# FaspDevTeam/faspsolver

Measured on AMD Instinct MI355X. Metric: AMG-PCG solve DOF/s (3D 7-pt Poisson 256^3, classical AMG V(1,1) w-Jacobi + PCG, rtol 1e-8), higher is better.
Workload: dtype f64

## Files before the change

### faspsolver_amd/__init__.py

```python
import ctypes as C
import os
import subprocess

import numpy as np

from . import _types as T
from ._types import *

_HERE = os.path.dirname(os.path.abspath(__file__))
LIB_PATH = os.environ.get("FASP_HIP_LIB") or os.path.join(_HERE, "libfasp_hip.so")
_lib = None

EXPORTS = [
    "fasp_param_amg_init", "fasp_param_solver_init", "fasp_solver_dcsr_krylov_amg",
    "fasp_blas_dcsr_mxv", "fasp_blas_dcsr_aAxpy", "fasp_blas_darray_dotprod",
    "fasp_blas_darray_norm2", "fasp_blas_darray_norminf", "fasp_blas_darray_axpy",
    "fasp_blas_darray_axpby", "fasp_smoother_dcsr_jacobi",
    "fasp_blas_dbsr_mxv", "fasp_blas_dbsr_aAxpy", "fasp_dbsr_getdiaginv", "fasp_smoother_dbsr_jacobi1",
    "fasp_solver_dbsr_pcg", "fasp_solver_dbsr_pbcgs", "fasp_solver_dbsr_pgmres", "fasp_solver_dbsr_pvgmres",
    "fasp_solver_dbsr_pvfgmres", "fasp_hip_bsr_precond_setup", "fasp_hip_bsr_precond_fct", "fasp_hip_bsr_precond_free",
    "fasp_hip_param_input", "fasp_fwrapper_dcsr_krylov_amg_", "fasp_dcsrvec_read2", "fasp_dvec_read",
    "fasp_dbsr_read", "fasp_dcoo_read", "fasp_dcoo_read1", "fasp_dcoo_shift_read", "fasp_dmtx_read", "fasp_dmtxsym_read", "fasp_dvec_write", "fasp_dcsr_write_coo", "fasp_dcsrvec_write2", "fasp_fwrapper_dcsr_amg_", "fasp_fwrapper_dbsr_krylov_amg_", "fasp_hip_free_bsr", "fasp_hip_comm_selftest", "fasp_hip_amg_kernel_info", "fasp_hip_coarse_kernel_info", "fasp_hip_bsr_coarse_kernel_info", "fasp_hip_coding_selftest", "fasp_solver_amg", "fasp_solver_famg", "fasp_hip_amg_solve", "fasp_precond_diag", "fasp_precond_dbsr_diag", "fasp_solver_dcsr_itsolver", "fasp_solver_dcsr_krylov", "fasp_solver_dcsr_krylov_diag", "fasp_solver_dbsr_itsolver", "fasp_solver_dbsr_krylov", "fasp_solver_dbsr_krylov_diag", "fasp_hip_mxv_csr", "fasp_hip_mxv_bsr", "fasp_solver_matfree_init", "fasp_solver_pcg", "fasp_solver_pbcgs", "fasp_solver_pgcg", "fasp_solver_pminres", "fasp_solver_pgmres", "fasp_solver_pvgmres", "fasp_solver_pvfgmres", "fasp_solver_itsolver", "fasp_solver_krylov", "fasp_solver_dcsr_pcg", "fasp_solver_dcsr_pminres", "fasp_solver_dcsr_pgcg", "fasp_solver_dcsr_pgcr", "fasp_solver_dcsr_pbcgs", "fasp_solver_dcsr_pgmres", "fasp_solver_dcsr_pvgmres",
    "fasp_solver_dcsr_pvfgmres", "fasp_hip_precond_setup", "fasp_hip_precond_fct", "fasp_hip_precond_free",
    "fasp_hip_time_bsr_mxv", "fasp_solver_dbsr_krylov_amg", "fasp_hip_bsr_amg_create", "fasp_hip_bsr_amg_create_host",
    "fasp_hip_bsr_amg_destroy", "fasp_hip_bsr_amg_num_levels", "fasp_hip_bsr_amg_get_matrix",
    "fasp_hip_bsr_amg_get_diaginv", "fasp_hip_bsr_solve",
    "fasp_hip_set_device", "fasp_hip_device_count", "fasp_hip_device_identity", "fasp_hip_available",
    "fasp_hip_amg_create", "fasp_hip_amg_create_host", "fasp_hip_amg_upload",
    "fasp_hip_amg_destroy", "fasp_hip_amg_num_levels", "fasp_hip_amg_get_matrix",
    "fasp_hip_amg_get_cfmark", "fasp_hip_solve", "fasp_hip_set_rhs", "fasp_hip_set_guess",
    "fasp_hip_solve_resident", "fasp_hip_get_solution", "fasp_hip_device_synchronize",
    "fasp_hip_precond_amg",
    "fasp_hip_poisson7pt", "fasp_hip_aniso27pt", "fasp_hip_free_system", "fasp_hip_time_kernel", "fasp_hip_measure_ceilings", "fasp_hip_amg_publish", "fasp_hip_amg_attach", "fasp_hip_amg_unpublish",
    "fasp_precond_setup", "fasp_precond_amg", "fasp_precond_famg", "fasp_precond_amli", "fasp_precond_namli", "fasp_amg_data_create", "fasp_amg_data_free", "fasp_param_amg_to_prec", "fasp_param_prec_to_amg", "fasp_mem_free", "fasp_mem_calloc", "fasp_dvec_alloc", "fasp_dvec_set", "fasp_dvec_free", "fasp_dvec_create", "fasp_dcsr_create", "fasp_dcsr_free", "fasp_smoother_dcsr_gs", "fasp_smoother_dcsr_sor", "fasp_smoother_dcsr_L1diag",
    "fasp_hip_tune", "fasp_hip_comm_unique_id", "fasp_hip_comm_init", "fasp_hip_comm_finalize",
    "fasp_hip_comm_rank", "fasp_hip_comm_size", "fasp_hip_version", "fasp_hip_comm_init_shm",
    "fasp_hip_dist_plan", "fasp_hip_dist_level_info", "fasp_hip_dist_get_matrix",
    "fasp_hip_dist_get_list",
    "fasp_blas_dcsr_vmv", "fasp_blas_dcsr_mxv_agg", "fasp_blas_dcsr_aAxpy_agg", "fasp_blas_darray_ax",
    "fasp_blas_darray_axpyz", "fasp_blas_darray_norm1", "fasp_darray_cp", "fasp_darray_set", "fasp_dvec_isnan",
    "fasp_hip_time_matrix", "fasp_hip_bsr_dist_info", "fasp_hip_seq_schedule_selftest", "fasp_hip_seq_chain_selftest", "fasp_hip_cluster_order", "fasp_hip_permute_csr", "fasp_hip_comm_init_ipc", "fasp_hip_comm_stats", "fasp_hip_comm_timing", "fasp_hip_estream_selftest", "fasp_hip_sell_selftest", "fasp_hip_csr_plan", "fasp_hip_level_op", "fasp_hip_matrix_op", "fasp_hip_matrix_traits",
    "fasp_param_ilu_init", "fasp_ilu_data_create", "fasp_ilu_data_free", "fasp_mem_iludata_check", "fasp_ilu_dcsr_setup",
    "fasp_precond_ilu", "fasp_precond_ilu_forward", "fasp_precond_ilu_backward", "fasp_solver_dcsr_krylov_ilu",
    "fasp_solver_dcsr_krylov_ilu_M", "fasp_smoother_dcsr_ilu", "fasp_fwrapper_dcsr_krylov_ilu_",
    "fasp_hip_ilu_resident_count", "fasp_hip_ilu_time",
    "fasp_ilu_dbsr_setup", "fasp_precond_dbsr_ilu", "fasp_solver_dbsr_krylov_ilu", "fasp_smoother_dbsr_ilu",
    "fasp_fwrapper_dbsr_krylov_ilu_",
    "fasp_hip_bsr_amg_get_ilu", "fasp_hip_bsr_amg_ilu_info", "fasp_hip_bsr_amg_ilu_smooth_time",
    "fasp_hip_bsr_sweep", "fasp_hip_csr_sweep",
    "fasp_blas_dcsr_rap", "fasp_hip_dcsr_rap", "fasp_hip_rap_info", "fasp_hip_rap_device_count", "fasp_hip_rap_time",
    "fasp_dstr_create", "fasp_dstr_alloc", "fasp_dstr_free", "fasp_dstr_cp", "fasp_format_dstr_dcsr", "fasp_dstr_read",
    "fasp_blas_dstr_aAxpy", "fasp_blas_dstr_mxv", "fasp_precond_dstr_diag", "fasp_solver_dstr_pcg", "fasp_solver_dstr_pbcgs",
    "fasp_solver_dstr_pminres", "fasp_solver_dstr_pgmres", "fasp_solver_dstr_pvgmres", "fasp_solver_dstr_itsolver",
    "fasp_solver_dstr_krylov", "fasp_solver_dstr_krylov_diag", "fasp_hip_mxv_str", "fasp_hip_str_form", "fasp_hip_time_str_mxv",
    "fasp_ilu_dstr_setup0", "fasp_ilu_dstr_setup1", "fasp_precond_dstr_ilu0", "fasp_precond_dstr_ilu1", "fasp_solver_dstr_krylov_ilu",
    "fasp_hip_str_ilu_form", "fasp_hip_str_ilu_apply", "fasp_hip_time_str_ilu",
    "fasp_smoother_dstr_jacobi", "fasp_smoother_dstr_jacobi1", "fasp_smoother_dstr_gs", "fasp_smoother_dstr_gs1",
    "fasp_smoother_dstr_gs_ascend", "fasp_smoother_dstr_gs_descend", "fasp_smoother_dstr_gs_order", "fasp_smoother_dstr_gs_cf",
    "fasp_smoother_dstr_sor", "fasp_smoother_dstr_sor1", "fasp_smoother_dstr_sor_ascend", "fasp_smoother_dstr_sor_descend",
    "fasp_smoother_dstr_sor_order", "fasp_smoother_dstr_sor_cf",
    "fasp_hip_str_sweep", "fasp_hip_str_sweep_form", "fasp_hip_str_sweep_levels", "fasp_hip_time_str_sweep",
    "fasp_generate_diaginv_block", "fasp_smoother_dstr_swz", "fasp_precond_dstr_blockgs", "fasp_solver_dstr_krylov_blockgs",
    "fasp_hip_str_swz", "fasp_hip_str_swz_levels", "fasp_hip_time_str_swz",
    "fasp_param_swz_init", "fasp_dcsr_sympart", "fasp_dcsr_shift", "fasp_sparse_mis", "fasp_swz_dcsr_setup", "fasp_dcsr_swz_forward",
    "fasp_dcsr_swz_backward", "fasp_precond_swz", "fasp_swz_data_free", "fasp_solver_dcsr_krylov_swz",
    "fasp_hip_csr_swz_levels", "fasp_hip_csr_swz", "fasp_hip_csr_swz_resident_count", "fasp_hip_time_csr_swz",
    "fasp_hip_csr_swz_runs", "fasp_hip_amg_get_swz", "fasp_hip_amg_swz_info", "fasp_hip_amg_swz_sweep_time", "fasp_hip_amg_swz_levels",
]


def build(verbose=False):
    cmd = ["make", "-C", os.path.join(_HERE, "csrc")]
    if not verbose:
        cmd.insert(1, "-s")
    subprocess.run(cmd, check=True)


def lib():
    global _lib
    if _lib is not None:
        return _lib
    if not os.path.exists(LIB_PATH):
        build()
    L = C.CDLL(LIB_PATH)
    P = C.POINTER
    L.fasp_param_amg_init.argtypes = [P(T.AMG_param)]
    L.fasp_param_solver_init.argtypes = [P(T.ITS_param)]
    L.fasp_solver_dcsr_krylov_amg.argtypes = [P(T.dCSRmat), P(T.dvector), P(T.dvector),
                                              P(T.ITS_param), P(T.AMG_param)]
    L.fasp_blas_dcsr_mxv.argtypes = [P(T.dCSRmat), T.c_double_p, T.c_double_p]
    L.fasp_blas_dcsr_aAxpy.argtypes = [C.c_double, P(T.dCSRmat), T.c_double_p, T.c_double_p]
    for f in ("fasp_blas_darray_dotprod", "fasp_blas_darray_norm2", "fasp_blas_darray_norminf"):
        getattr(L, f).restype = C.c_double
    L.fasp_blas_darray_dotprod.argtypes = [C.c_int, T.c_double_p, T.c_double_p]
    L.fasp_blas_darray_norm2.argtypes = [C.c_int, T.c_double_p]
    L.fasp_blas_darray_norminf.argtypes = [C.c_int, T.c_double_p]
    L.fasp_blas_darray_axpy.argtypes = [C.c_int, C.c_double, T.c_double_p, T.c_double_p]
    L.fasp_blas_darray_axpby.argtypes = [C.c_int, C.c_double, T.c_double_p, C.c_double,
                                         T.c_double_p]
    L.fasp_blas_dcsr_vmv.restype = C.c_double
    L.fasp_blas_dcsr_vmv.argtypes = [P(T.dCSRmat), T.c_double_p, T.c_double_p]
    L.fasp_blas_dcsr_mxv_agg.argtypes = [P(T.dCSRmat), T.c_double_p, T.c_double_p]
    L.fasp_blas_dcsr_aAxpy_agg.argtypes = [C.c_double, P(T.dCSRmat), T.c_double_p, T.c_double_p]
    L.fasp_blas_darray_ax.argtypes = [C.c_int, C.c_double, T.c_double_p]
    L.fasp_blas_darray_axpyz.argtypes = [C.c_int, C.c_double, T.c_double_p, T.c_double_p, T.c_double_p]
    L.fasp_blas_darray_norm1.restype = C.c_double
    L.fasp_blas_darray_norm1.argtypes = [C.c_int, T.c_double_p]
    L.fasp_darray_cp.argtypes = [C.c_int, T.c_double_p, T.c_double_p]
    L.fasp_darray_set.argtypes = [C.c_int, T.c_double_p, C.c_double]
    L.fasp_hip_time_matrix.restype = C.c_double
    L.fasp_hip_time_matrix.argtypes = [P(T.dCSRmat), C.c_int, C.c_int, P(C.c_int)]
    L.fasp_dvec_isnan.restype = C.c_short
    L.fasp_dvec_isnan.argtypes = [P(T.dvector)]
    L.fasp_smoother_dcsr_jacobi.argtypes = [P(T.dvector), C.c_int, C.c_int, C.c_int,
                                            P(T.dCSRmat), P(T.dvector), C.c_int, C.c_double]
    L.fasp_blas_dbsr_mxv.argtypes = [P(T.dBSRmat), T.c_double_p, T.c_double_p]
    L.fasp_blas_dbsr_aAxpy.argtypes = [C.c_double, P(T.dBSRmat), T.c_double_p, T.c_double_p]
    L.fasp_dbsr_getdiaginv.argtypes = [P(T.dBSRmat)]
    L.fasp_dbsr_getdiaginv.restype = T.dvector
    L.fasp_smoother_dbsr_jacobi1.argtypes = [P(T.dBSRmat), P(T.dvector), P(T.dvector), T.c_double_p]
    L.fasp_hip_bsr_sweep.argtypes = [P(T.dBSRmat), T.c_double_p, T.c_double_p, T.c_double_p, C.c_int, C.c_int, C.c_double,
                                     P(C.c_int)]
    L.fasp_hip_csr_sweep.argtypes = [P(T.dCSRmat), P(C.c_int), C.c_int, C.c_int, C.c_double, C.c_int, T.c_double_p, T.c_double_p,
                                     P(C.c_int)]
    L.fasp_hip_time_bsr_mxv.argtypes = [P(T.dBSRmat), C.c_int]
    L.fasp_hip_time_bsr_mxv.restype = C.c_double
    L.fasp_solver_dcsr_pcg.argtypes = [P(T.dCSRmat), P(T.dvector), P(T.dvector), P(T.precond), C.c_double,
                                       C.c_double, C.c_int, C.c_short, C.c_short]
    L.fasp_solver_dcsr_pbcgs.argtypes = L.fasp_solver_dcsr_pcg.argtypes
    L.fasp_solver_dcsr_pminres.argtypes = L.fasp_solver_dcsr_pcg.argtypes
    L.fasp_solver_dcsr_pgcg.argtypes = L.fasp_solver_dcsr_pcg.argtypes
    L.fasp_solver_dcsr_pvgmres.argtypes = [P(T.dCSRmat), P(T.dvector), P(T.dvector), P(T.precond), C.c_double,
                                           C.c_double, C.c_int, C.c_short, C.c_short, C.c_short]
    L.fasp_solver_dcsr_pvfgmres.argtypes = L.fasp_solver_dcsr_pvgmres.argtypes
    L.fasp_solver_dcsr_pgmres.argtypes = L.fasp_solver_dcsr_pvgmres.argtypes
    L.fasp_solver_dcsr_pgcr.argtypes = L.fasp_solver_dcsr_pvgmres.argtypes
    L.fasp_hip_precond_setup.argtypes = [P(T.dCSRmat), P(T.AMG_param)]
    L.fasp_hip_precond_setup.restype = P(T.precond)
    L.fasp_hip_precond_free.argtypes = [P(T.precond)]
    L.fasp_hip_precond_free.restype = None
    L.fasp_hip_precond_fct.argtypes = [T.c_double_p, T.c_double_p, C.c_void_p]
    L.fasp_hip_precond_fct.restype = None
    L.fasp_solver_dbsr_pcg.argtypes = [P(T.dBSRmat), P(T.dvector), P(T.dvector), P(T.precond), C.c_double,
                                       C.c_double, C.c_int, C.c_short, C.c_short]
    L.fasp_solver_dbsr_pbcgs.argtypes = L.fasp_solver_dbsr_pcg.argtypes
    L.fasp_solver_dbsr_pvgmres.argtypes = [P(T.dBSRmat), P(T.dvector), P(T.dvector), P(T.precond), C.c_double,
                                           C.c_double, C.c_int, C.c_short, C.c_short, C.c_short]
    L.fasp_solver_dbsr_pgmres.argtypes = L.fasp_solver_dbsr_pvgmres.argtypes
    L.fasp_solver_dbsr_pvfgmres.argtypes = L.fasp_solver_dbsr_pvgmres.argtypes
    L.fasp_hip_bsr_precond_setup.argtypes = [P(T.dBSRmat), P(T.AMG_param)]
    L.fasp_hip_bsr_precond_setup.restype = P(T.precond)
    L.fasp_hip_bsr_precond_free.argtypes = [P(T.precond)]
    L.fasp_hip_bsr_precond_free.restype = None
    L.fasp_hip_bsr_precond_fct.argtypes = [T.c_double_p, T.c_double_p, C.c_void_p]
    L.fasp_hip_bsr_precond_fct.restype = None
    L.fasp_dcsrvec_read2.argtypes = [C.c_char_p, C.c_char_p, P(T.dCSRmat), P(T.dvector)]
    L.fasp_dvec_read.argtypes = [C.c_char_p, P(T.dvector)]
    L.fasp_dbsr_read.argtypes = [C.c_char_p, P(T.dBSRmat)]
    L.fasp_hip_free_bsr.argtypes = [P(T.dBSRmat)]
    L.fasp_hip_free_bsr.restype = None
    L.fasp_hip_param_input.argtypes = [C.c_char_p, P(T.ITS_param), P(T.AMG_param)]
    L.fasp_fwrapper_dcsr_krylov_amg_.argtypes = [P(C.c_int), P(C.c_int), T.c_int_p, T.c_int_p, T.c_double_p,
                                                 T.c_double_p, T.c_double_p, P(C.c_double), P(C.c_int), P(C.c_int)]
    L.fasp_fwrapper_dcsr_krylov_amg_.restype = None
    L.fasp_hip_coding_selftest.argtypes = [P(T.dCSRmat), P(C.c_int)]
    L.fasp_hip_amg_kernel_info.argtypes = [C.c_void_p, C.c_int, C.c_int, P(C.c_int), P(C.c_double)]
    L.fasp_hip_coarse_kernel_info.argtypes = [C.c_void_p, P(C.c_int)]
    L.fasp_hip_bsr_coarse_kernel_info.argtypes = [C.c_void_p, P(C.c_int)]
    L.fasp_solver_amg.argtypes = [P(T.dCSRmat), P(T.dvector), P(T.dvector), P(T.AMG_param)]
    L.fasp_hip_amg_solve.argtypes = [C.c_void_p, P(T.dvector), P(T.dvector), P(T.AMG_param), T.c_double_p,
                                     C.c_int, P(T.fasp_hip_stats)]
    L.fasp_solver_dbsr_krylov_amg.argtypes = [P(T.dBSRmat), P(T.dvector), P(T.dvector), P(T.ITS_param),
                                              P(T.AMG_param)]
    L.fasp_hip_bsr_amg_create.argtypes = [P(C.c_void_p), P(T.dBSRmat), P(T.AMG_param)]
    L.fasp_hip_bsr_amg_create_host.argtypes = [P(C.c_void_p), P(T.dBSRmat), P(T.AMG_param)]
    L.fasp_hip_bsr_amg_destroy.argtypes = [C.c_void_p]
    L.fasp_hip_bsr_amg_destroy.restype = None
    L.fasp_hip_bsr_amg_num_levels.argtypes = [C.c_void_p]
    L.fasp_hip_bsr_amg_get_matrix.argtypes = [C.c_void_p, C.c_int, C.c_int, P(T.dBSRmat)]
    L.fasp_hip_bsr_amg_get_diaginv.argtypes = [C.c_void_p, C.c_int]
    L.fasp_hip_bsr_amg_get_diaginv.restype = T.c_double_p
    L.fasp_hip_bsr_solve.argtypes = [C.c_void_p, P(T.dvector), P(T.dvector), P(T.ITS_param), T.c_double_p,
                                     C.c_int, P(T.fasp_hip_stats)]
    L.fasp_hip_amg_create.argtypes = [P(C.c_void_p), P(T.dCSRmat), P(T.AMG_param)]
    L.fasp_hip_amg_create_host.argtypes = L.fasp_hip_amg_create.argtypes
    L.fasp_hip_amg_upload.argtypes = [C.c_void_p]
    L.fasp_hip_amg_destroy.argtypes = [C.c_void_p]
    L.fasp_hip_amg_destroy.restype = None
    L.fasp_hip_amg_num_levels.argtypes = [C.c_void_p]
    L.fasp_hip_amg_get_matrix.argtypes = [C.c_void_p, C.c_int, C.c_int, P(T.dCSRmat)]
    L.fasp_hip_amg_get_cfmark.argtypes = [C.c_void_p, C.c_int, P(T.ivector)]
    L.fasp_hip_solve.argtypes = [C.c_void_p, P(T.dvector), P(T.dvector), P(T.ITS_param),
                                 T.c_double_p, C.c_int, P(T.fasp_hip_stats)]
    L.fasp_hip_set_rhs.argtypes = [C.c_void_p, P(T.dvector)]
    L.fasp_hip_set_guess.argtypes = [C.c_void_p, P(T.dvector)]
    L.fasp_hip_get_solution.argtypes = [C.c_void_p, P(T.dvector)]
    L.fasp_hip_solve_resident.argtypes = [C.c_void_p, P(T.ITS_param), T.c_double_p, C.c_int,
                                          P(T.fasp_hip_stats)]
    L.fasp_hip_precond_amg.argtypes = [C.c_void_p, T.c_double_p, T.c_double_p]
    L.fasp_hip_poisson7pt.argtypes = [C.c_int, C.c_int, C.c_int, P(T.dCSRmat), P(T.dvector),
                                      P(T.dvector)]
    L.fasp_hip_aniso27pt.argtypes = [C.c_int, C.c_double, C.c_double, C.c_double, P(T.dCSRmat), P(T.dvector)]
    L.fasp_hip_free_system.argtypes = [P(T.dCSRmat), P(T.dvector), P(T.dvector)]
    L.fasp_hip_free_system.restype = None
    L.fasp_hip_measure_ceilings.argtypes = [P(C.c_double), C.c_size_t, C.c_int]
    L.fasp_hip_amg_publish.argtypes = [C.c_void_p, C.c_char_p]
    L.fasp_hip_amg_attach.argtypes = [P(C.c_void_p), C.c_char_p]
    L.fasp_hip_amg_unpublish.argtypes = [C.c_char_p]
    L.fasp_hip_time_kernel.restype = C.c_double
    L.fasp_hip_time_kernel.argtypes = [C.c_void_p, C.c_int, C.c_int, C.c_int]
    L.fasp_hip_tune.argtypes = [C.c_char_p, C.c_int]
    L.fasp_hip_comm_unique_id.argtypes = [C.c_char_p]
    L.fasp_hip_comm_init.argtypes = [C.c_int, C.c_int, C.c_char_p]
    L.fasp_hip_version.restype = C.c_char_p
    L.fasp_hip_comm_init_shm.argtypes = [C.c_int, C.c_int, C.c_char_p]
    L.fasp_hip_dist_plan.argtypes = [C.c_void_p, C.c_int, C.c_int, C.c_int]
    L.fasp_hip_dist_level_info.argtypes = [C.c_void_p, C.c_int, T.c_int_p]
    L.fasp_hip_dist_get_matrix.argtypes = [C.c_void_p, C.c_int, C.c_int, P(T.dCSRmat)]
    L.fasp_hip_dist_get_list.argtypes = [C.c_void_p, C.c_int, C.c_int, P(T.ivector)]
    _lib = L
    L.fasp_param_ilu_init.argtypes = [P(T.ILU_param)]
    L.fasp_param_ilu_init.restype = None
    L.fasp_ilu_data_create.argtypes = [C.c_int, C.c_int, P(T.ILU_data)]
    L.fasp_ilu_data_create.restype = None
    L.fasp_ilu_data_free.argtypes = [P(T.ILU_data)]
    L.fasp_ilu_data_free.restype = None
    L.fasp_mem_iludata_check.argtypes = [P(T.ILU_data)]
    L.fasp_mem_iludata_check.restype = C.c_short
    L.fasp_ilu_dcsr_setup.argtypes = [P(T.dCSRmat), P(T.ILU_data), P(T.ILU_param)]
    L.fasp_ilu_dcsr_setup.restype = C.c_short
    for f in ("fasp_precond_ilu", "fasp_precond_ilu_forward", "fasp_precond_ilu_backward"):
        getattr(L, f).argtypes = [T.c_double_p, T.c_double_p, C.c_void_p]
        getattr(L, f).restype = None
    L.fasp_solver_dcsr_krylov_ilu.argtypes = [P(T.dCSRmat), P(T.dvector), P(T.dvector), P(T.ITS_param), P(T.ILU_param)]
    L.fasp_solver_dcsr_krylov_ilu_M.argtypes = [P(T.dCSRmat), P(T.dvector), P(T.dvector), P(T.ITS_param),
                                                P(T.ILU_param), P(T.dCSRmat)]
    L.fasp_smoother_dcsr_ilu.argtypes = [P(T.dCSRmat), P(T.dvector), P(T.dvector), C.c_void_p]
    L.fasp_smoother_dcsr_ilu.restype = None
    L.fasp_fwrapper_dcsr_krylov_ilu_.argtypes = [P(C.c_int), P(C.c_int), T.c_int_p, T.c_int_p, T.c_double_p,
                                                 T.c_double_p, T.c_double_p, P(C.c_double), P(C.c_int), P(C.c_int)]
    L.fasp_fwrapper_dcsr_krylov_ilu_.restype = None
    L.fasp_hip_ilu_time.argtypes = [P(T.ILU_data), C.c_int, C.c_int, T.c_double_p]
    L.fasp_hip_ilu_time.restype = C.c_double
    L.fasp_ilu_dbsr_setup.argtypes = [P(T.dBSRmat), P(T.ILU_data), P(T.ILU_param)]
    L.fasp_ilu_dbsr_setup.restype = C.c_short
    L.fasp_precond_dbsr_ilu.argtypes = [T.c_double_p, T.c_double_p, C.c_void_p]
    L.fasp_precond_dbsr_ilu.restype = None
    L.fasp_solver_dbsr_krylov_ilu.argtypes = [P(T.dBSRmat), P(T.dvector), P(T.dvector), P(T.ITS_param), P(T.ILU_param)]
    L.fasp_solver_dbsr_krylov_ilu.restype = C.c_int
# ... 264 lines not shown
    def publish(self, name):
        st = lib().fasp_hip_amg_publish(self.h, name.encode())
        if st < 0:
            raise RuntimeError(f"fasp_hip_amg_publish({name}) failed with status {st}")

    @staticmethod
    def unpublish(name):
        lib().fasp_hip_amg_unpublish(name.encode())

    @property
    def num_levels(self):
        return lib().fasp_hip_amg_num_levels(self.h)

    def upload(self):
        st = lib().fasp_hip_amg_upload(self.h)
        if st < 0:
            raise RuntimeError(f"fasp_hip_amg_upload failed with status {st}")

    def matrix(self, level, which):
        v = T.dCSRmat()
        st = lib().fasp_hip_amg_get_matrix(self.h, level, which, C.byref(v))
        if st < 0:
            raise IndexError((level, which))
        ia, ja, val = T.csr_arrays(v)
        return v.row, v.col, ia, ja, val

    def cfmark(self, level):
        v = T.ivector()
        if lib().fasp_hip_amg_get_cfmark(self.h, level, C.byref(v)) < 0:
            raise IndexError(level)
        return np.ctypeslib.as_array(v.val, (v.row,)).copy()

    def solve(self, b, itparam, x0=None, hist_cap=600):
        x = np.zeros(self.n) if x0 is None else np.ascontiguousarray(x0, dtype=np.float64).copy()
        bv, _b = T.as_vec(b)
        xv, x = T.as_vec(x)
        hist = np.zeros(hist_cap)
        stats = T.fasp_hip_stats()
        st = lib().fasp_hip_solve(self.h, C.byref(bv), C.byref(xv), C.byref(itparam),
                                  T.dp(hist), hist_cap, C.byref(stats))
        return st, x, hist[:max(stats.nhist, 0)].copy(), stats

    def amg_solve(self, b, amgparam=None, x0=None, hist_cap=600):
        x = np.zeros(self.n) if x0 is None else np.ascontiguousarray(x0, dtype=np.float64).copy()
        bv, _b = T.as_vec(b)
        xv, x = T.as_vec(x)
        hist = np.zeros(hist_cap)
        stats = T.fasp_hip_stats()
        st = lib().fasp_hip_amg_solve(self.h, C.byref(bv), C.byref(xv),
                                      C.byref(amgparam) if amgparam is not None else None,
                                      T.dp(hist), hist_cap, C.byref(stats))
        return st, x, hist[:max(min(stats.nhist, hist_cap), 0)].copy(), stats

    def set_rhs(self, b):
        bv, _b = T.as_vec(b)
        st = lib().fasp_hip_set_rhs(self.h, C.byref(bv))
        if st < 0:
            raise RuntimeError(f"fasp_hip_set_rhs failed: {st}")

    def solve_resident(self, itparam, hist_cap=600):
        st = lib().fasp_hip_set_guess(self.h, None)
        if st < 0:
            raise RuntimeError(f"fasp_hip_set_guess failed: {st}")
        hist = np.zeros(hist_cap)
        stats = T.fasp_hip_stats()
        st = lib().fasp_hip_solve_resident(self.h, C.byref(itparam), T.dp(hist), hist_cap,
                                           C.byref(stats))
        return st, hist[:max(stats.nhist, 0)].copy(), stats

    def get_solution(self):
        x = np.zeros(self.n)
        xv, x = T.as_vec(x)
        st = lib().fasp_hip_get_solution(self.h, C.byref(xv))
        if st < 0:
            raise RuntimeError(f"fasp_hip_get_solution failed: {st}")
        return x

    def kernel_info(self, level, which=0):
        k = C.c_int(0); b = C.c_double(0)
        if lib().fasp_hip_amg_kernel_info(self.h, level, which, C.byref(k), C.byref(b)) < 0:
            raise IndexError((level, which))
        return k.value, b.value

    def coarse_kernel_info(self):
        info = (C.c_int * 8)()
        if lib().fasp_hip_coarse_kernel_info(self.h, info) < 0:
            raise RuntimeError("fasp_hip_coarse_kernel_info failed")
        return tuple(info)

    def precond(self, r):
        r = np.ascontiguousarray(r, dtype=np.float64)
        z = np.zeros_like(r)
        st = lib().fasp_hip_precond_amg(self.h, T.dp(r), T.dp(z))
        if st < 0:
            raise RuntimeError(f"fasp_hip_precond_amg failed: {st}")
        return z

    def dist_plan(self, rank, nranks, min_rows):
        st = lib().fasp_hip_dist_plan(self.h, rank, nranks, min_rows)
        if st < 0:
            raise RuntimeError(f"fasp_hip_dist_plan failed: {st}")

    def dist_info(self, level):
        info = (C.c_int * 8)()
        if lib().fasp_hip_dist_level_info(self.h, level, info) < 0:
            raise IndexError(level)
        keys = ("replicated", "nglobal", "row0", "nloc", "nghost", "nsend", "first_replicated", "nranks")
        return dict(zip(keys, list(info)))

    def dist_matrix(self, level, which):
        v = T.dCSRmat()
        if lib().fasp_hip_dist_get_matrix(self.h, level, which, C.byref(v)) < 0:
            raise IndexError((level, which))
        ia, ja, val = T.csr_arrays(v)
        return v.row, v.col, ia, ja, val

    def dist_list(self, level, which):
        v = T.ivector()
        if lib().fasp_hip_dist_get_list(self.h, level, which, C.byref(v)) < 0:
            raise IndexError((level, which))
        if v.row == 0:
            return np.zeros(0, np.int32)
        return np.ctypeslib.as_array(v.val, (v.row,)).copy()

    def time_kernel(self, kind, level=0, reps=20):
        return lib().fasp_hip_time_kernel(self.h, kind, level, reps)

    def swz(self, level):
        d = T.SWZ_data()
        st = lib().fasp_hip_amg_get_swz(self.h, level, C.byref(d))
        if st < 0:
            raise IndexError(level)
        if st == 0:
            return None
        iblock = np.ctypeslib.as_array(d.iblock, (d.nblk + 1,)).copy()
        jblock = np.ctypeslib.as_array(d.jblock, (int(iblock[-1]),)).copy()
        n, nnz = d.A.row, d.A.nnz
        ia = np.ctypeslib.as_array(d.A.IA, (n + 1,)).copy()
        ja = np.ctypeslib.as_array(d.A.JA, (max(nnz, 1),))[:nnz].copy()
        val = np.ctypeslib.as_array(d.A.val, (max(nnz, 1),))[:nnz].copy()
        return dict(nblk=d.nblk, maxbs=d.maxbs, SWZ_type=d.SWZ_type, iblock=iblock, jblock=jblock, A=(ia, ja, val))

    def swz_levels(self, level):
        v = C.c_int(0)
        if lib().fasp_hip_amg_swz_levels(self.h, level, C.byref(v)) < 0:
            raise IndexError(level)
        return v.value

    def swz_info(self, level):
        info = (C.c_int * 8)()
        st = lib().fasp_hip_amg_swz_info(self.h, level, info)
        if st < 0:
            raise IndexError(level)
        if st == 0:
            return None
        keys = ("levels_fwd", "levels_bwd", "launches_fwd", "launches_bwd", "nblk", "maxbs", "nswap", "nfactor")
        return dict(zip(keys, list(info)))

    def swz_sweep_time(self, level, dir=0, reps=20):
        ms = lib().fasp_hip_amg_swz_sweep_time(self.h, level, dir, reps)
        if ms < 0:
            raise RuntimeError(f"fasp_hip_amg_swz_sweep_time failed: {int(ms)}")
        return ms

    def close(self):
        if self.h:
# ... 121 lines not shown
```

### faspsolver_amd/csrc/device_csr.hip.h

```cpp

struct DevCSR {
    int     row = 0, col = 0, nnz = 0;
    int*    ia  = nullptr;
    int*    ja  = nullptr;
    double* val = nullptr;
    int*    dpos = nullptr;
    bool    dup_diag = false;
    bool    sorted = false;
    int     lanes = 8;
    int     kind = 0;
    int     tile_rows = 256;
    int     wrows = 64, wcap = 512;
    unsigned char* code = nullptr;
    int*    rowbase = nullptr;
    int*    doff = nullptr;
    double* dval = nullptr;
    unsigned short* pat = nullptr;
    int*    pstart = nullptr;
    int*    plen = nullptr;
    int*    poff = nullptr;
    double* pval = nullptr;
    int     npat = 0, npent = 0;
    unsigned short* ja16 = nullptr;
    int*            jbase = nullptr;
    int     nxrows = -1;
    int     plane = 0;
    int     win_lo = 0, win_hi = -1;
    unsigned short* lja16 = nullptr;
    int*    tptr = nullptr;
    int*    tcols = nullptr;
    long long ntcols = 0;
    const int* bridge = nullptr;
    double*    bscratch = nullptr;
    int        bridge_dir = 0;
    int*       es_tab = nullptr;
    unsigned short* es_ja16 = nullptr;
    double*    es_part = nullptr;
    int        es_W = 0, es_nc = 0;
    unsigned*      sell_code = nullptr;
    int*           sell_meta = nullptr;
    unsigned char* sell_rlen = nullptr;
    double*        sell_tab = nullptr;
    int            sell_nv = 0, sell_obits = 0, sell_nslice = 0;
    long long      sell_slots = 0;
    void    release()
    {
        if (sell_code) (void)hipFree(sell_code);
        if (sell_meta) (void)hipFree(sell_meta);
        if (sell_rlen) (void)hipFree(sell_rlen);
        if (sell_tab) (void)hipFree(sell_tab);
        sell_code = nullptr; sell_meta = nullptr; sell_rlen = nullptr; sell_tab = nullptr; sell_nv = sell_obits = sell_nslice = 0; sell_slots = 0;
        if (es_tab) (void)hipFree(es_tab);
        if (es_part) (void)hipFree(es_part);
        if (es_ja16) (void)hipFree(es_ja16);
        es_tab = nullptr; es_part = nullptr; es_ja16 = nullptr; es_W = es_nc = 0;
        if (bscratch) (void)hipFree(bscratch);
        bscratch = nullptr; bridge = nullptr; bridge_dir = 0;
        if (lja16) (void)hipFree(lja16);
        if (tptr) (void)hipFree(tptr);
        if (tcols) (void)hipFree(tcols);
        lja16 = nullptr; tptr = nullptr; tcols = nullptr;
        nxrows = -1;
        if (ja16) (void)hipFree(ja16);
        ja16 = nullptr;
        if (jbase) (void)hipFree(jbase);
        jbase = nullptr;
        if (ia) (void)hipFree(ia);
        if (ja) (void)hipFree(ja);
        if (val) (void)hipFree(val);
        if (dpos) (void)hipFree(dpos);
        if (code) (void)hipFree(code);
        if (rowbase) (void)hipFree(rowbase);
        if (doff) (void)hipFree(doff);
        if (dval) (void)hipFree(dval);
        if (pat) (void)hipFree(pat);
        if (pstart) (void)hipFree(pstart);
        if (plen) (void)hipFree(plen);
        if (poff) (void)hipFree(poff);
        if (pval) (void)hipFree(pval);
        pat = nullptr; pstart = plen = poff = nullptr; pval = nullptr;
        ia = ja = dpos = rowbase = doff = nullptr; val = dval = nullptr; code = nullptr;
    }
};

static void pick_kernel(DevCSR& M)
{
    const double avg = M.row > 0 ? (double)M.nnz / M.row : 1.0;
    static const double stream_max = std::getenv("FASP_HIP_STREAM_MAX") ? std::atof(std::getenv("FASP_HIP_STREAM_MAX")) : 48.0;
    M.kind = avg <= stream_max ? 2 : 0;
    M.lanes = avg < 300.0 ? 16 : avg < 1000.0 ? 32 : 64;
    while (M.lanes < 64 && (double)M.row * M.lanes < 0.75 * MAXGRID * BLOCK) M.lanes *= 2;
    if (avg < 48.0) M.lanes = avg < 3.0 ? 2 : avg < 6.0 ? 4 : avg < 24.0 ? 8 : 16;
    static const int small_rows = std::getenv("FASP_HIP_SMALL_XFER_ROWS") ? std::atoi(std::getenv("FASP_HIP_SMALL_XFER_ROWS")) : 256 * 1024;
    if (M.kind == 2 && M.row != M.col && M.row < small_rows) M.kind = 0;
    int R = 256;
    while (R < STREAM_MAXR && R * 2 * avg <= 3072.0) R <<= 1;
    M.tile_rows = R;
    M.wrows = 64;
    M.wcap  = 512;
}

static bool g_oneshot_upload = false;
static bool compress_enabled()
{
    if (g_oneshot_upload) return false;
    static int en = -1;
    if (en < 0) { const char* e = std::getenv("FASP_HIP_COMPRESS"); en = (e && std::atoi(e) == 0) ? 0 : 1; }
    return en != 0;
}
struct PairKey { int off; unsigned long long bits; };
static inline unsigned pair_hash(int off, unsigned long long bits)
{
    unsigned long long h = bits * 0x9E3779B97F4A7C15ull + (unsigned long long)(unsigned)off * 0xC2B2AE3D27D4EB4Full;
    return (unsigned)(h >> 40);
}
static bool build_dict8(const HostCSR& M, std::vector<int>& doff, std::vector<double>& dval,
                        Buf<unsigned char>& code, Buf<int>& rowbase)
{
    const bool square = M.row == M.col;
    const int n = M.row;
    if (n <= 0 || M.nnz <= 0) return false;
    constexpr int SLOTS = 1024;
    struct Table {
        int      cnt = 0;
        int      slot_id[SLOTS];
        PairKey  keys[257];
        Table() { for (int& s : slot_id) s = -1; }
        int find_or_add(int off, unsigned long long bits, bool add)
        {
// ... 127 lines not shown
#pragma omp for schedule(static)
        for (int r = 0; r < n; ++r) {
            const unsigned long long h = row_hash(r);
            rh[r] = h;
            if (fail) continue;
            S->add(h, r);
            if (S->cnt > maxpat) fail = true;
        }
    }
    Set* Gs = nullptr;
    std::vector<std::pair<int, unsigned long long>> reps;
    if (!fail) {
        Gs = new Set(SLOTS);
        for (Set* S : local)
            if (S)
                for (int s = 0; s < SLOTS && !fail; ++s)
                    if (S->key[s]) { Gs->add(S->key[s], S->first[s]); if (Gs->cnt > maxpat) fail = true; }
    }
    for (Set* S : local) delete S;
    if (fail) { delete Gs; return false; }
    for (int s = 0; s < SLOTS; ++s)
        if (Gs->key[s]) reps.emplace_back(Gs->first[s], Gs->key[s]);
    std::sort(reps.begin(), reps.end());
    long long tot = 0;
    for (auto& q : reps) tot += (M.ia[q.first + 1] - M.ia[q.first] + 7) / 8 * 8;
    if (tot > MAXENT || (long long)reps.size() * 8 > n || tot * 4 > M.nnz) { delete Gs; return false; }
    pstart.assign(reps.size(), 0); plen.assign(reps.size(), 0);
    poff.clear(); pval.clear();
    for (size_t i = 0; i < reps.size(); ++i) {
        const int r = reps[i].first, base = base_of(r);
        pstart[i] = (int)poff.size();
        plen[i] = M.ia[r + 1] - M.ia[r];
        for (int k = M.ia[r]; k < M.ia[r + 1]; ++k) { poff.push_back(M.ja[k] - base); pval.push_back(M.val[k]); }
        while (poff.size() % 8) { poff.push_back(0); pval.push_back(0.0); }
    }
    for (int s = 0; s < SLOTS; ++s) Gs->first[s] = -1;
    {
        Set& S = *Gs;
        for (size_t i = 0; i < reps.size(); ++i) {
            unsigned s = (unsigned)(reps[i].second >> 20) & (SLOTS - 1);
            while (S.key[s] != reps[i].second) s = (s + 1) & (SLOTS - 1);
            S.first[s] = (int)i;
        }
    }
    pat.alloc((size_t)n);
    if (!square) rowbase.alloc((size_t)n);
    bool collision = false;
#pragma omp parallel for schedule(static) num_threads(nt)
    for (int r = 0; r < n; ++r) {
        const int id = Gs->find(rh[r]);
        if (id < 0 || !same_row(r, reps[(size_t)id].first)) { collision = true; continue; }
        pat[r] = (unsigned short)id;
        if (!square) rowbase[r] = base_of(r);
    }
    delete Gs;
    return !collision;
}

static int grid_plane_of(const std::vector<int>& poff, int nrow)
{
    constexpr int UNIT = 8 * 2 * BLOCK;
    std::vector<int> cand;
    for (int o : poff) {
        const long long m = std::llabs((long long)o);
        const long long c = (m + UNIT / 2) / UNIT * UNIT;
        if (c >= UNIT && c <= nrow / 4 && std::find(cand.begin(), cand.end(), (int)c) == cand.end() && cand.size() < 64) cand.push_back((int)c);
    }
    int best = 0;
    double best_cost = 0.2;
    for (int P : cand) {
        double cost = 0.0;
        for (int o : poff) {
            long long r = (long long)o % P;
            if (r > P / 2) r -= P;
            if (r < -P / 2) r += P;
            cost += (double)std::min<long long>(std::llabs(r), P / 8) / (P / 8);
        }
        cost /= std::max<size_t>(poff.size(), 1);
        if (cost < best_cost || (cost == best_cost && P > best)) { best_cost = cost; best = P; }
    }
    return best;
}

static bool rows_span_16bit(const int* ia, const int* ja, int row)
{
    int bad = 0;
#pragma omp parallel for schedule(static) reduction(+ : bad)
    for (int i = 0; i < row; ++i) {
        if (ia[i + 1] <= ia[i]) continue;
        int lo = ja[ia[i]], hi = lo;
        for (int k = ia[i] + 1; k < ia[i + 1]; ++k) { lo = std::min(lo, ja[k]); hi = std::max(hi, ja[k]); }
        if (hi - lo >= 65536) ++bad;
    }
    return bad == 0;
}
static int upload_ja16(DevCSR& D, const int* ia_host, const int* ja_dev_order)
{
    static const bool on = !(std::getenv("FASP_HIP_JA16") && std::atoi(std::getenv("FASP_HIP_JA16")) == 0);
    if (!on || D.kind != 0 || D.nnz < 4096) return FASP_SUCCESS;
    const bool relative = D.col > 65536;
    if (relative && !rows_span_16bit(ia_host, ja_dev_order, D.row)) return FASP_SUCCESS;
    Buf<unsigned short> j16((size_t)D.nnz);
    Buf<int> base(relative ? (size_t)D.row : 0);
#pragma omp parallel for schedule(static)
    for (int i = 0; i < D.row; ++i) {
        int lo = 0;
        if (relative) {
            lo = ia_host[i + 1] > ia_host[i] ? ja_dev_order[ia_host[i]] : 0;
            for (int k = ia_host[i]; k < ia_host[i + 1]; ++k) lo = std::min(lo, ja_dev_order[k]);
            base[(size_t)i] = lo;
        }
        for (int k = ia_host[i]; k < ia_host[i + 1]; ++k) j16[k] = (unsigned short)(ja_dev_order[k] - lo);
    }
    HIPCK(hipMalloc(&D.ja16, sizeof(unsigned short) * ((size_t)D.nnz + 8)));
    HIPCK(hipMemset(D.ja16 + D.nnz, 0, sizeof(unsigned short) * 8));
    HIPCK(hipMemcpy(D.ja16, j16.data(), sizeof(unsigned short) * (size_t)D.nnz, hipMemcpyHostToDevice));
    if (relative) {
        HIPCK(hipMalloc(&D.jbase, sizeof(int) * (size_t)D.row));
        HIPCK(hipMemcpy(D.jbase, base.data(), sizeof(int) * (size_t)D.row, hipMemcpyHostToDevice));
    }
    return FASP_SUCCESS;
}

static int g_device_sort = 1;
constexpr int SORT_BLK = 256, SORT_MAXLEN = 16384;
__global__ __launch_bounds__(SORT_BLK) void k_sort_rows(int nrow, const int* __restrict__ ia, const int* __restrict__ ja_in,
                                                        const double* __restrict__ val_in, int* __restrict__ ja_out,
                                                        double* __restrict__ val_out, unsigned short* __restrict__ ja16, int* __restrict__ jbase)
{
    extern __shared__ unsigned long long sort_keys[];
    const int tid = threadIdx.x;
    for (int r = blockIdx.x; r < nrow; r += gridDim.x) {
        const int kb = ia[r], len = ia[r + 1] - kb;
        int P = 1;
        while (P < len) P <<= 1;
        for (int i = tid; i < P; i += SORT_BLK)
            sort_keys[i] = i < len ? ((unsigned long long)(unsigned)ja_in[kb + i] << 32) | (unsigned)i : ~0ull;
        __syncthreads();
        for (int k = 2; k <= P; k <<= 1)
            for (int j = k >> 1; j > 0; j >>= 1) {
                for (int t = tid; t < P / 2; t += SORT_BLK) {
                    const int i = ((t & ~(j - 1)) << 1) | (t & (j - 1)), l = i | j;
                    const unsigned long long a = sort_keys[i], b = sort_keys[l];
                    if ((a > b) == ((i & k) == 0)) { sort_keys[i] = b; sort_keys[l] = a; }
                }
                __syncthreads();
            }
        const int base = (jbase && len > 0) ? (int)(sort_keys[0] >> 32) : 0;
        if (jbase && tid == 0) jbase[r] = base;
        for (int i = tid; i < len; i += SORT_BLK) {
            const unsigned long long key = sort_keys[i];
            const int col = (int)(key >> 32);
            ja_out[kb + i] = col;
            val_out[kb + i] = val_in[kb + (int)(unsigned)key];
            if (ja16) ja16[kb + i] = (unsigned short)(col - base);
        }
        __syncthreads();
    }
}

static int upload_sorted_on_device(const HostCSR& H, DevCSR& D, int maxlen)
{
    static const bool ja16_on = !(std::getenv("FASP_HIP_JA16") && std::atoi(std::getenv("FASP_HIP_JA16")) == 0);
    int* tj = nullptr; double* tv = nullptr;
    HIPCK(hipMalloc(&tj, sizeof(int) * (size_t)H.nnz));
    if (hipMalloc(&tv, sizeof(double) * (size_t)H.nnz) != hipSuccess) { (void)hipFree(tj); return ERROR_ALLOC_MEM; }
// ... 357 lines not shown
#pragma omp parallel for schedule(static)
    for (int s = 0; s < ns; ++s) {
        const int W = S.sptr[(size_t)s + 1] - S.sptr[(size_t)s], base = S.sbase[(size_t)s];
        unsigned* cs = S.code.data() + (size_t)S.sptr[(size_t)s] * 64;
        for (int l = 0; l < 64; ++l) {
            const int r = s * 64 + l;
            const int kb = r < n ? M.ia[r] : 0, len = r < n ? M.ia[r + 1] - kb : 0;
            for (int k = 0; k < len; ++k) {
                const int sl = Gs.slot(bits_of(M.val[kb + k]));
                if (sl < 0) { lost = true; continue; }
                const int id = Gs.id[(size_t)sl];
                cs[(size_t)k * 64 + l] = ((unsigned)id << S.obits) | (unsigned)(M.ja[kb + k] - base);
            }
            for (int k = len; k < W; ++k) cs[(size_t)k * 64 + l] = 0u;
        }
    }
    if (lost) { why = 4; return false; }
    why = 0;
    return true;
}

static void sell_mxv_host(const SellHost& S, int nrow, const double* x, double* y)
{
    const unsigned omask = (1u << S.obits) - 1u;
    for (int s = 0; s < S.nslice; ++s) {
        const int W = S.sptr[(size_t)s + 1] - S.sptr[(size_t)s], base = S.sbase[(size_t)s];
        const unsigned* cs = S.code.data() + (size_t)S.sptr[(size_t)s] * 64;
        double acc[64];
        for (int l = 0; l < 64; ++l) acc[l] = 0.0;
        for (int k = 0; k < W; ++k)
            for (int l = 0; l < 64; ++l) {
                const int r = s * 64 + l;
                if (r >= nrow || k >= (int)S.rlen[(size_t)r]) continue;
                const unsigned c = cs[(size_t)k * 64 + l];
                acc[l] = acc[l] + S.tab[c >> S.obits] * x[base + (int)(c & omask)];
            }
        for (int l = 0; l < 64 && s * 64 + l < nrow; ++l) y[s * 64 + l] = acc[l];
    }
}
static void sell_decode_host(const SellHost& S, int nrow, int* ia, int* ja, double* val)
{
    const unsigned omask = (1u << S.obits) - 1u;
    ia[0] = 0;
    for (int r = 0; r < nrow; ++r) ia[r + 1] = ia[r] + (int)S.rlen[(size_t)r];
    for (int r = 0; r < nrow; ++r) {
        const int s = r >> 6, l = r & 63, base = S.sbase[(size_t)s];
        const unsigned* cs = S.code.data() + (size_t)S.sptr[(size_t)s] * 64;
        for (int k = 0; k < (int)S.rlen[(size_t)r]; ++k) {
            const unsigned c = cs[(size_t)k * 64 + l];
            ja[ia[r] + k] = base + (int)(c & omask);
            val[ia[r] + k] = S.tab[c >> S.obits];
        }
    }
}

static int upload_sell(const HostCSR& H, DevCSR& D)
{
    static const bool on = !(std::getenv("FASP_HIP_SELL") && std::atoi(std::getenv("FASP_HIP_SELL")) == 0);
    if (!on) return FASP_SUCCESS;
    static const bool timing = std::getenv("FASP_HIP_SETUP_TIMING") != nullptr;
    const double t0 = wall_seconds();
    SellHost S;
    int why = 0;
    const bool ok = build_sell(H, S, SELL_CAP_PERCENT, &why);
    if (timing) std::printf("        [sell %d x %d, %d nnz] %s (%d) %d values, %d + %d bits, %.3f slots per entry, %.3f s\n", H.row, H.col, H.nnz,
                            ok ? "coded" : "not coded", why, S.nv, S.vbits, S.obits, (double)S.slots / std::max(H.nnz, 1), wall_seconds() - t0);
    if (!ok) return FASP_SUCCESS;
    const size_t ns = (size_t)S.nslice;
    std::vector<int> meta(2 * ns + 1);
    std::copy(S.sptr.begin(), S.sptr.end(), meta.begin());
    std::copy(S.sbase.begin(), S.sbase.end(), meta.begin() + (long)ns + 1);
    HIPCK(hipMalloc(&D.sell_code, sizeof(unsigned) * (size_t)std::max<long long>(S.slots, 1)));
    HIPCK(hipMalloc(&D.sell_meta, sizeof(int) * meta.size()));
    HIPCK(hipMalloc(&D.sell_rlen, (size_t)H.row));
    HIPCK(hipMalloc(&D.sell_tab, sizeof(double) * (size_t)S.nv));
    HIPCK(hipMemcpy(D.sell_code, S.code.data(), sizeof(unsigned) * (size_t)S.slots, hipMemcpyHostToDevice));
    HIPCK(hipMemcpy(D.sell_meta, meta.data(), sizeof(int) * meta.size(), hipMemcpyHostToDevice));
    HIPCK(hipMemcpy(D.sell_rlen, S.rlen.data(), (size_t)H.row, hipMemcpyHostToDevice));
    HIPCK(hipMemcpy(D.sell_tab, S.tab.data(), sizeof(double) * (size_t)S.nv, hipMemcpyHostToDevice));
    D.sell_nv = S.nv; D.sell_obits = S.obits; D.sell_nslice = S.nslice; D.sell_slots = S.slots;
    return FASP_SUCCESS;
}

static int upload_csr(const HostCSR& H, DevCSR& D)
{
    D.row = H.row; D.col = H.col; D.nnz = H.nnz;
    HIPCK(hipMalloc(&D.ia, sizeof(int) * ((size_t)H.row + 1)));
    HIPCK(hipMalloc(&D.ja, sizeof(int) * std::max<size_t>(H.nnz, 1)));
    HIPCK(hipMalloc(&D.val, sizeof(double) * (std::max<size_t>(H.nnz, 1) + 2)));
    HIPCK(hipMemsetAsync(D.val + std::max<size_t>(H.nnz, 1), 0, sizeof(double) * 2, g_ctx.stream));
    HIPCK(hipMemcpyAsync(D.ia, H.ia.data(), sizeof(int) * ((size_t)H.row + 1), hipMemcpyHostToDevice, g_ctx.stream));
    pick_kernel(D);
    auto upload_plain = [&]() -> int {
        HIPCK(hipMemcpyAsync(D.ja, H.ja.data(), sizeof(int) * (size_t)H.nnz, hipMemcpyHostToDevice, g_ctx.stream));
        HIPCK(hipMemcpyAsync(D.val, H.val.data(), sizeof(double) * (size_t)H.nnz, hipMemcpyHostToDevice, g_ctx.stream));
        return 0;
    };
    if (compress_enabled() && H.nnz >= 4096 && (double)H.nnz <= 48.0 * H.row) {
        Buf<unsigned short> pat; Buf<int> prb;
        std::vector<int> pstart, plen, poff; std::vector<double> pval;
        static const bool rowpat_on = !(std::getenv("FASP_HIP_ROWPAT") && std::atoi(std::getenv("FASP_HIP_ROWPAT")) == 0);
        if (rowpat_on && build_rowpat(H, pat, pstart, plen, poff, pval, prb)) {
            D.npat = (int)pstart.size(); D.npent = (int)poff.size();
            HIPCK(hipMalloc(&D.pat, sizeof(unsigned short) * ((size_t)H.row + 2)));
            HIPCK(hipMalloc(&D.pstart, sizeof(int) * pstart.size()));
            HIPCK(hipMalloc(&D.plen, sizeof(int) * plen.size()));
            HIPCK(hipMemcpy(D.plen, plen.data(), sizeof(int) * plen.size(), hipMemcpyHostToDevice));
            HIPCK(hipMalloc(&D.poff, sizeof(int) * std::max<size_t>(poff.size(), 1)));
            HIPCK(hipMalloc(&D.pval, sizeof(double) * std::max<size_t>(pval.size(), 1)));
            HIPCK(hipMemset(D.pat + H.row, 0xff, sizeof(unsigned short) * 2));
            HIPCK(hipMemcpy(D.pat, pat.data(), sizeof(unsigned short) * (size_t)H.row, hipMemcpyHostToDevice));
            HIPCK(hipMemcpy(D.pstart, pstart.data(), sizeof(int) * pstart.size(), hipMemcpyHostToDevice));
            HIPCK(hipMemcpy(D.poff, poff.data(), sizeof(int) * poff.size(), hipMemcpyHostToDevice));
            HIPCK(hipMemcpy(D.pval, pval.data(), sizeof(double) * pval.size(), hipMemcpyHostToDevice));
            if (prb.n) {
                HIPCK(hipMalloc(&D.rowbase, sizeof(int) * ((size_t)H.row + 2)));
                HIPCK(hipMemcpy(D.rowbase, prb.data(), sizeof(int) * (size_t)H.row, hipMemcpyHostToDevice));
                const int nr = H.row, npair = (nr + 1) / 2;
                long long nx = 0;
#pragma omp parallel for schedule(static) reduction(+ : nx)
                for (int w0 = 0; w0 < nr; w0 += 128) {
                    const int    pm = std::min((w0 + 64) / 2, npair - 1);
                    const unsigned domA = pat[(size_t)2 * pm], domB = (2 * pm + 1 < nr) ? pat[(size_t)2 * pm + 1] : 0xffffu;
                    for (int r = w0; r < std::min(w0 + 128, nr); r += 2) {
                        const bool vb = r + 1 < nr;
                        if (!(vb && pat[r] == domA && pat[r + 1] == domB)) nx += vb ? 2 : 1;
                    }
                }
                if (nx * 4 <= nr) D.nxrows = (int)nx;
            } else {
                D.plane = grid_plane_of(poff, H.row);
                if (std::getenv("FASP_HIP_SETUP_TIMING")) std::printf("        [upload_csr %d x %d, %d nnz] %d row patterns; grid plane for the XCD strips: %d rows\n", H.row, H.col, H.nnz, (int)pstart.size(), D.plane);
                const int nr = H.row, npair = (nr + 1) / 2;
                long long nx = 0;
#pragma omp parallel for schedule(static) reduction(+ : nx)
                for (int w0 = 0; w0 < nr; w0 += 128) {
                    const unsigned dom = pat[(size_t)2 * std::min((w0 + 64) / 2, npair - 1)];
                    for (int r = w0; r < std::min(w0 + 128, nr); r += 2) {
                        const bool vb = r + 1 < nr;
                        if (!(vb && pat[r] == dom && pat[r + 1] == dom)) nx += vb ? 2 : 1;
                    }
                }
                if (nx * 4 <= nr) D.nxrows = (int)nx;
            }
            D.kind = 2;
            return upload_plain() < 0 ? ERROR_ALLOC_MEM : FASP_SUCCESS;
        }
        std::vector<int> doff; std::vector<double> dval;
        Buf<unsigned char> code; Buf<int> rowbase;
        if (build_dict8(H, doff, dval, code, rowbase)) {
            HIPCK(hipMalloc(&D.code, (size_t)H.nnz + 256));
            HIPCK(hipMalloc(&D.doff, sizeof(int) * 256));
            HIPCK(hipMalloc(&D.dval, sizeof(double) * 256));
            HIPCK(hipMemcpy(D.code, code.data(), (size_t)H.nnz, hipMemcpyHostToDevice));
            HIPCK(hipMemcpy(D.doff, doff.data(), sizeof(int) * 256, hipMemcpyHostToDevice));
            HIPCK(hipMemcpy(D.dval, dval.data(), sizeof(double) * 256, hipMemcpyHostToDevice));
            if (rowbase.n) {
                HIPCK(hipMalloc(&D.rowbase, sizeof(int) * (size_t)H.row));
                HIPCK(hipMemcpy(D.rowbase, rowbase.data(), sizeof(int) * (size_t)H.row, hipMemcpyHostToDevice));
            }
            D.kind = 2;
            return upload_plain() < 0 ? ERROR_ALLOC_MEM : FASP_SUCCESS;
        }
    }
    static const bool sort_long = !(std::getenv("FASP_HIP_SORT_LONG_ROWS") && std::atoi(std::getenv("FASP_HIP_SORT_LONG_ROWS")) == 0);
    static const int  sort_stream = std::getenv("FASP_HIP_SORT_STREAM") ? std::atoi(std::getenv("FASP_HIP_SORT_STREAM")) : 0;
    const double avg_len = H.row > 0 ? (double)H.nnz / H.row : 0.0;
    const bool do_sort = sort_long && !g_oneshot_upload && H.nnz > 0 && (D.kind == 0 || (D.kind == 2 && sort_stream > 0 && avg_len >= sort_stream));
    static const bool timing = std::getenv("FASP_HIP_SETUP_TIMING") != nullptr;
    double tp = wall_seconds();
    auto lap = [&](const char* what) {
        if (!timing) return;
        const double now = wall_seconds();
        std::printf("        [upload_csr %d x %d, %d nnz] %-10s %8.3f s\n", H.row, H.col, H.nnz, what, now - tp);
        tp = now;
    };
    if (do_sort && D.kind == 0) {
        int maxlen = 0;
#pragma omp parallel for schedule(static) reduction(max : maxlen)
        for (int i = 0; i < H.row; ++i) maxlen = std::max(maxlen, H.ia[i + 1] - H.ia[i]);
        if (g_device_sort && maxlen <= SORT_MAXLEN) {
            const int st = upload_sorted_on_device(H, D, maxlen);
            lap("device sort");
            return st < 0 ? st : build_estream(H.ia.data(), H.row, H.nnz, D);
        }
    }
    if (do_sort) {
        Buf<int> sj((size_t)H.nnz);
        Buf<double> sv((size_t)H.nnz);
        std::vector<int> dp;
        const bool square = H.row == H.col;
        if (square) dp.assign((size_t)H.row, -1);
#pragma omp parallel
        {
            std::vector<std::pair<int, double>> tmp;
#pragma omp for schedule(dynamic, 64)
            for (int i = 0; i < H.row; ++i) {
                const int kb = H.ia[i], ke = H.ia[i + 1];
                tmp.resize((size_t)(ke - kb));
                for (int k = kb; k < ke; ++k) tmp[(size_t)(k - kb)] = {H.ja[k], H.val[k]};
                std::stable_sort(tmp.begin(), tmp.end(),
                                 [](const std::pair<int, double>& x, const std::pair<int, double>& y) { return x.first < y.first; });
                for (int k = kb; k < ke; ++k) {
                    sj[k] = tmp[(size_t)(k - kb)].first; sv[k] = tmp[(size_t)(k - kb)].second;
                    if (square && sj[k] == i) dp[(size_t)i] = k;
                }
            }
        }
        lap("row sort");
        HIPCK(hipMemcpy(D.ja, sj.data(), sizeof(int) * (size_t)H.nnz, hipMemcpyHostToDevice));
        HIPCK(hipMemcpy(D.val, sv.data(), sizeof(double) * (size_t)H.nnz, hipMemcpyHostToDevice));
        lap("memcpy");
        if (square && D.kind == 2) {
            HIPCK(hipMalloc(&D.dpos, sizeof(int) * (size_t)std::max(H.row, 1)));
            HIPCK(hipMemcpy(D.dpos, dp.data(), sizeof(int) * (size_t)H.row, hipMemcpyHostToDevice));
        }
        D.sorted = true;
        if (upload_ja16(D, H.ia.data(), sj.data()) < 0) return ERROR_ALLOC_MEM;
        return build_estream(H.ia.data(), H.row, H.nnz, D);
    }
    if (upload_plain() < 0) return ERROR_ALLOC_MEM;
    if (D.kind == 2 && !g_oneshot_upload && build_xtile(H, D) < 0) return ERROR_ALLOC_MEM;
    if (D.kind == 2 && compress_enabled() && upload_sell(H, D) < 0) return ERROR_ALLOC_MEM;
    if (upload_ja16(D, H.ia.data(), H.ja.data()) < 0) return ERROR_ALLOC_MEM;
    return build_estream(H.ia.data(), H.row, H.nnz, D);
}

struct Tuning { int swz_run = -1, swz_run_width = 16, ilu_smooth_fused = 1, gen2 = 2, ws2_bpc = 3, maxgrid = -1, xcd = 16, nt = 1, kind = -1, lanes = -1, wrows = -1, wcap = -1, compress = 1, rpl = -1, lds_tab = 1, xcd_pat = 64, spcg_batch = 16, small_lds = 1, ja16 = 1, spcg_fused = 1, spcg_grid = 0, spcg_persist = 1, split_rows = 0, gs_multicolor = 0, seq_flow = 1, seq_strip_kb = 0, seq_jobs = 1, seq_spine = 1, seq_grid = 0, seq_chain = 1, seq_chain_n1 = 0, seq_chain_grid = 0, seq_chain_ref = 0, seq_test_hang = 0, seq_rest_lanes = 0, local_square = 1, fuse_zr = 1, fuse_presmooth = 1, seq_lanes = 0, xtile = 1, rp5_max = 45, rp_bpc = 5, rp_xcd = -1, rp_strip = 2, spcg_test_hang = 0, small_onewave = 4, lazy_coarse = 1, rp_stream = -1, renumber = 1, renumber_chunk = 262144, pcg_dev_beta = 1, spcg_spec = 1, ev_every = 4, pcg_fold = 1, seq_chain_touch = 8, seq_chain_touch_t1 = 1, seq_zero_skip = 1, estream = 1, es_dbg = 0, ilu_form = -1, str_ilu_form = -1, str_ilu_wgs = 0, str_sweep_form = -1, str_sweep_wgs = 0, sell = 1; };
static Tuning g_tune;

template <class K>
static int resident_blocks_per_cu(K kernel)
{
    static std::vector<std::pair<const void*, int>> cache;
    const void* key = reinterpret_cast<const void*>(kernel);
    for (const auto& e : cache)
        if (e.first == key) return e.second;
    int nb = 0;
    if (hipOccupancyMaxActiveBlocksPerMultiprocessor(&nb, kernel, BLOCK, 0) != hipSuccess || nb < 1) nb = 4;
    nb = std::min(nb, 8);
    cache.emplace_back(key, nb);
    return nb;
}

template <class K>
static int launch_persistent(K kernel, int ntiles, CsrArgs& a, int blocks_per_cu = 0)
{
    int cap = (blocks_per_cu > 0 ? std::min(blocks_per_cu, resident_blocks_per_cu(kernel)) : resident_blocks_per_cu(kernel)) * g_ctx.num_cu;
    if (g_tune.maxgrid > 0) cap = g_tune.maxgrid;
    cap = std::min(cap, MAXGRID);
    int grid = std::min(cap, ntiles);
    grid = std::max(8, (grid + 7) / 8 * 8);
    hipLaunchKernelGGL(kernel, dim3(grid), dim3(BLOCK), 0, g_ctx.stream, a);
    return grid;
}

enum CsrKernel : int {
    CK_ROWS_2 = 0, CK_ROWS_4, CK_ROWS_8, CK_ROWS_16, CK_ROWS_32, CK_ROWS_64,
    CK_WSTREAM_64_512, CK_WSTREAM_64_1024, CK_WSTREAM_32_512, CK_WSTREAM_32_1024,
    CK_ROWPAT_0_1, CK_ROWPAT_0_2, CK_ROWPAT_1_1, CK_ROWPAT_1_2, CK_ROWPAT_2_1, CK_ROWPAT_2_2,
    CK_DICT8_8, CK_DICT8_16, CK_DICT8_24,
    CK_ESTREAM_4, CK_ESTREAM_8, CK_ESTREAM_16, CK_ESTREAM_32,
    CK_ROWPAT4, CK_ROWPAT5, CK_LSTREAM, CK_XTILE, CK_SELL, CK_WSTREAM2
};
struct CsrPlan {
    CsrKernel kernel;
    int    family;
    int    tile_rows;
    int    bpc;
    int    xcd_map;
    int    tpp;
    int    nt;
    bool   ja16, jbase;
    bool   fused_zr;
    double bytes;
};
static CsrPlan plan_csr(const DevCSR& M, int op, bool windowed, bool want_partials, int rows = -1)
{
    CsrPlan p{};
    int kind = M.kind;
    if (rows < 0) rows = M.row;
    if (M.code && g_tune.compress) kind = 4;
    if (M.pat && g_tune.compress) kind = 5;
    if (g_tune.kind >= 0 && !(g_tune.kind == 4 && !M.code) && !(g_tune.kind == 5 && !M.pat)) kind = g_tune.kind;
    const int lanes = g_tune.lanes > 0 ? g_tune.lanes : M.lanes, wrows = g_tune.wrows > 0 ? g_tune.wrows : M.wrows, wcap = g_tune.wcap > 0 ? g_tune.wcap : M.wcap;
    const bool jac = op == OP_JACOBI, w64 = wrows == 64 && wcap == 512;
    const bool lstream_ok = g_tune.gen2 && kind == 2 && w64 && (double)M.nnz <= 7.6 * M.row;
    if (jac && kind != 0 && kind < 4 && (M.dup_diag || !M.dpos) && !lstream_ok) kind = 0;
    p.xcd_map = g_tune.xcd;
    p.nt = g_tune.nt | ((g_tune.rp_stream > 0 || (g_tune.rp_stream < 0 && (size_t)M.row * 8 > (size_t)96 << 20)) ? 4 : 0);
    p.ja16 = g_tune.ja16 && M.ja16; p.jbase = g_tune.ja16 && M.jbase;
    if (M.jbase && kind != 0) p.ja16 = p.jbase = false;
    if (kind == 1 || kind == 3) kind = 0;
    p.tile_rows = kind >= 4 ? BLOCK : kind == 2 ? 4 * wrows : BLOCK / lanes;
    auto ntiles = [&] { return (rows + p.tile_rows - 1) / p.tile_rows; };
    auto strips = [&] {
        const int rpb = p.tile_rows;
        if (!g_tune.rp_strip || M.plane < 8 * rpb || M.plane % (8 * rpb) != 0 || ntiles() < 4 * (M.plane / rpb)) return;
        p.xcd_map = -2; p.tpp = M.plane / rpb;
    };
    const double avg = M.row > 0 ? (double)M.nnz / M.row : 1.0, ptr_bytes = 4.0 * (M.row + 1.0), base_bytes = M.rowbase ? 4.0 * M.row : 0.0;
    const bool pair = kind == 5 && M.nxrows >= 0 && g_tune.rpl <= 0;
    p.bytes = kind == 5 ? 2.0 * M.row + base_bytes + 12.0 * M.npent : kind == 4 ? 1.0 * M.nnz + ptr_bytes + base_bytes : 12.0 * M.nnz + ptr_bytes;
    if (pair && g_tune.gen2 && !M.rowbase) {
        p.kernel = CK_ROWPAT4; p.family = 6; p.tile_rows = 2 * BLOCK;
        p.xcd_map = ntiles() >= 8 * 64 ? g_tune.rp_xcd : 16;
        if (p.xcd_map == -1) strips();
        p.bpc = p.xcd_map == -2 && g_tune.rp_bpc == 5 ? 3 : g_tune.rp_bpc;
        p.fused_zr = jac && want_partials;
    }
    else if (pair && g_tune.gen2 >= 2 && M.rowbase && !jac && op != OP_L1DIAG && (double)M.nnz <= 0.1 * g_tune.rp5_max * M.row) {
        p.kernel = CK_ROWPAT5; p.family = 9; p.tile_rows = 2 * BLOCK; p.bpc = 5;
        p.xcd_map = ntiles() >= 8 * 64 ? -1 : 16;
        if (g_tune.rp_strip >= 2) strips();
    }
    else if (kind == 5) {
        const int rpl = g_tune.rpl > 0 ? g_tune.rpl : 1;
        const bool lds = M.npat <= 512 && M.npent <= 2048 && g_tune.lds_tab != 0;
        const int T = !lds ? 0 : M.npat <= 64 && M.npent <= 512 && g_tune.lds_tab != 3 ? 2 : 1;
        p.kernel = CsrKernel(CK_ROWPAT_0_1 + 2 * T + (rpl != 1)); p.family = 5; p.tile_rows = BLOCK * rpl;
        if (g_tune.xcd_pat != 0) p.xcd_map = g_tune.xcd_pat;
        if (g_tune.xcd_pat == 64 && g_tune.rp_strip >= 2) strips();
    }
    else if (kind == 4) { p.kernel = avg <= 8.5 ? CK_DICT8_8 : avg <= 20.0 ? CK_DICT8_16 : CK_DICT8_24; p.family = 4; }
    else if (lstream_ok) { p.kernel = CK_LSTREAM; p.family = 7; p.bpc = 4; p.fused_zr = jac && want_partials; }
    else if (kind == 2 && g_tune.gen2 >= 2 && w64) {
        if (g_tune.xtile && M.lja16) {
            p.kernel = CK_XTILE; p.family = 10; p.bpc = 3;
            p.bytes = 10.0 * M.nnz + ptr_bytes + 4.0 * M.ntcols + 4.0 * ((M.row + 63) / 64 + 1.0);
        }
        else if (M.sell_code && g_tune.compress && g_tune.sell) {
            p.kernel = CK_SELL; p.family = 11; p.tile_rows = SELL_BLOCK;
            p.bytes = 4.0 * (double)M.sell_slots + 1.0 * M.row + 4.0 * (2.0 * M.sell_nslice + 1.0) + 8.0 * M.sell_nv;
        }
        else { p.kernel = CK_WSTREAM2; p.family = 8; p.bpc = g_tune.ws2_bpc; }
        p.fused_zr = jac && want_partials;
    }
    else if (kind == 2) {
        p.kernel = w64 ? CK_WSTREAM_64_512 : wrows == 64 ? CK_WSTREAM_64_1024 : wrows == 32 && wcap == 512 ? CK_WSTREAM_32_512 : CK_WSTREAM_32_1024; p.family = 2;
    }
    else {
        if (p.ja16) p.bytes = 10.0 * M.nnz + ptr_bytes + (p.jbase ? 4.0 * M.row : 0.0);
        const bool es_rule = g_tune.estream >= 2 || (g_tune.estream == 1 && (double)M.nnz < 256.0 * M.row);
        if (M.es_tab && es_rule && p.ja16 && !windowed && op != OP_MXV_DOT && !(jac && (want_partials || M.dup_diag)))
            p.kernel = avg >= 512.0 ? CK_ESTREAM_32 : avg >= 256.0 ? CK_ESTREAM_16 : avg >= 128.0 ? CK_ESTREAM_8 : CK_ESTREAM_4;
        else
            p.kernel = lanes == 2 ? CK_ROWS_2 : lanes == 4 ? CK_ROWS_4 : lanes == 8 ? CK_ROWS_8 : lanes == 16 ? CK_ROWS_16 : lanes == 32 ? CK_ROWS_32 : CK_ROWS_64;
    }
    return p;
}
static int kernel_family(const DevCSR& M, double* matrix_bytes)
{
    const CsrPlan p = plan_csr(M, OP_MXV, false, false);
    if (matrix_bytes) *matrix_bytes = p.bytes;
    return p.family;
}

template <int OP>
static int launch_sell(const DevCSR& M, CsrArgs& a)
{
    a.sell_code = M.sell_code; a.sell_sptr = M.sell_meta; a.sell_sbase = M.sell_meta + M.sell_nslice + 1; a.sell_rlen = M.sell_rlen;
    a.sell_tab = M.sell_tab; a.sell_nv = M.sell_nv; a.sell_obits = M.sell_obits;
    const size_t lds = sizeof(double) * ((size_t)M.sell_nv + SELL_NW);
    static bool attr_set = false;
    if (!attr_set) {
        (void)hipFuncSetAttribute(reinterpret_cast<const void*>(k_csr_sell<OP>), hipFuncAttributeMaxDynamicSharedMemorySize, (int)(sizeof(double) * (SELL_MAXV + SELL_NW)));
        attr_set = true;
    }
    static std::vector<std::pair<size_t, int>> cache;
    int nb = 0;
    for (const auto& e : cache)
        if (e.first == lds) nb = e.second;
    if (nb == 0) {
        if (hipOccupancyMaxActiveBlocksPerMultiprocessor(&nb, k_csr_sell<OP>, SELL_BLOCK, lds) != hipSuccess || nb < 1) nb = 1;
        nb = std::min(nb, 2);
        cache.emplace_back(lds, nb);
    }
    int cap = nb * g_ctx.num_cu;
    if (g_tune.maxgrid > 0) cap = g_tune.maxgrid;
    cap = std::min(cap, MAXGRID);
    int grid = std::min(cap, a.ntiles);
    grid = std::max(8, (grid + 7) / 8 * 8);
    hipLaunchKernelGGL(k_csr_sell<OP>, dim3(grid), dim3(SELL_BLOCK), lds, g_ctx.stream, a);
    return grid;
}

template <int OP>
static int launch_rowpat5(CsrArgs& a)
{
    if constexpr (OP == OP_JACOBI || OP == OP_L1DIAG) { (void)a; return 0; }
    else return launch_persistent(k_csr_rowpat5<OP>, a.ntiles, a, 5);
}

constexpr int WIN_ALIGN = DIST_WIN_ALIGN;
struct RowWin { int lo = 0, hi = -1, goff = 0; };

__global__ __launch_bounds__(BLOCK) void k_bridge_gather(int n, const int* __restrict__ perm, const double* __restrict__ s, double* __restrict__ y,
                                                         double* __restrict__ zx, const double* __restrict__ zdiag, double zomega)
{
    for (int k = blockIdx.x * BLOCK + threadIdx.x; k < n; k += gridDim.x * BLOCK) {
        const double v = s[perm[k]];
        y[k] = v;
        if (zx) { const double di = zdiag[k]; zx[k] = (fabs(di) > 1e-20) ? (1 - zomega) * 0.0 + zomega * v / di : 0.0; }
    }
}
__global__ __launch_bounds__(BLOCK) void k_bridge_scatter(int n, const int* __restrict__ perm, const double* __restrict__ x, double* __restrict__ s)
{
    for (int k = blockIdx.x * BLOCK + threadIdx.x; k < n; k += gridDim.x * BLOCK) s[perm[k]] = x[k];
}

template <int OP>
static int launch_csr(const DevCSR& M0, CsrArgs a, RowWin win = RowWin())
{
    if (M0.bridge && win.hi < 0) {
        DevCSR Mn = M0;
        Mn.bridge = nullptr; Mn.bscratch = nullptr; Mn.bridge_dir = 0;
        if (M0.bridge_dir == 1 && OP == OP_MXV) {
            CsrArgs b = a;
            b.y = M0.bscratch; b.zx = nullptr; b.zdiag = nullptr;
            const int G = launch_csr<OP>(Mn, b);
            const int grid = std::max(1, std::min(MAXGRID, (M0.row + BLOCK - 1) / BLOCK));
            hipLaunchKernelGGL(k_bridge_gather, dim3(grid), dim3(BLOCK), 0, g_ctx.stream, M0.row, M0.bridge, (const double*)M0.bscratch, a.y, a.zx, a.zdiag, a.zomega);
            return G;
        }
        if (M0.bridge_dir == 2 && (OP == OP_ADD || OP == OP_SUB || OP == OP_AXPY || OP == OP_MXV)) {
            const int grid = std::max(1, std::min(MAXGRID, (M0.col + BLOCK - 1) / BLOCK));
            hipLaunchKernelGGL(k_bridge_scatter, dim3(grid), dim3(BLOCK), 0, g_ctx.stream, M0.col, M0.bridge, a.x, M0.bscratch);
            CsrArgs b = a;
            b.x = M0.bscratch;
            return launch_csr<OP>(Mn, b);
        }
        std::fprintf(stderr, "### ERROR: fasp_hip: operation %d on a transfer operator with a numbering bridge (direction %d)\n", (int)OP, M0.bridge_dir);
        std::abort();
    }
    if (win.hi < 0 && g_tune.split_rows > 0 && M0.row >= 4 * WIN_ALIGN) {
        const int lo = std::min(g_tune.split_rows, M0.row / 4) / WIN_ALIGN * WIN_ALIGN, hi = (M0.row - lo) / WIN_ALIGN * WIN_ALIGN;
        RowWin w; w.lo = lo; w.hi = hi; w.goff = 0;
        int G = launch_csr<OP>(M0, a, w);
        w.lo = 0; w.hi = lo; w.goff = G;
        G += launch_csr<OP>(M0, a, w);
        w.lo = hi; w.hi = M0.row; w.goff = G;
        return G + launch_csr<OP>(M0, a, w);
    }
    const DevCSR& M = M0;
    const int w_lo = win.hi >= 0 ? win.lo : 0, w_hi = win.hi >= 0 ? std::min(win.hi, M0.row) : M0.row;
    if (w_hi <= w_lo && win.hi >= 0) return 0;
    if (a.partials) a.partials += win.goff;
    const CsrPlan p = plan_csr(M, OP, win.hi >= 0 || g_tune.split_rows > 0, a.partials != nullptr, w_hi - w_lo);
    const int rpb = p.tile_rows;
    if (win.hi >= 0 && rpb > 0 && (w_lo % rpb) != 0) {
        std::fprintf(stderr, "### ERROR: fasp_hip: row window at %d with a kernel tile of %d rows (a tuning knob broke the window alignment)\n", w_lo, rpb);
        std::abort();
    }
    a.nrow = w_hi; a.row_lo = w_lo; a.tile0 = w_lo / rpb;
    a.ntiles = (w_hi - w_lo + rpb - 1) / rpb; a.tiles_per_xcd = (a.ntiles + 7) / 8;
    a.xcd_map = p.xcd_map; a.nt = p.nt;
    if (p.tpp) { a.tpp = p.tpp; a.tiles_per_xcd = p.tpp / 8; }
    a.ia = M.ia; a.ja = M.ja; a.val = M.val; a.dpos = M.dpos;
    a.ja16 = p.ja16 ? M.ja16 : nullptr; a.jbase = p.jbase ? M.jbase : nullptr;
    if (p.family == 5 || p.family == 6 || p.family == 9) {
        a.pat = M.pat; a.pstart = M.pstart; a.plen = M.plen; a.poff = M.poff; a.pval = M.pval; a.rowbase = M.rowbase;
        a.npat = M.npat; a.npent = M.npent; a.ncol = M.col;
    }
    if (p.family == 4) { a.code = M.code; a.rowbase = M.rowbase; a.doff = M.doff; a.dval = M.dval; }
    if (p.kernel == CK_XTILE) { a.lja16 = M.lja16; a.tptr = M.tptr; a.tcols = M.tcols; }
#define PERSIST(...) return launch_persistent(__VA_ARGS__, a.ntiles, a, p.bpc)
    switch (p.kernel) {
        case CK_ROWS_2:  PERSIST(k_csr_rows<2, OP>);
        case CK_ROWS_4:  PERSIST(k_csr_rows<4, OP>);
        case CK_ROWS_8:  PERSIST(k_csr_rows<8, OP>);
        case CK_ROWS_16: PERSIST(k_csr_rows<16, OP>);
        case CK_ROWS_32: PERSIST(k_csr_rows<32, OP>);
        case CK_ROWS_64: PERSIST(k_csr_rows<64, OP>);
        case CK_WSTREAM_64_512:  PERSIST(k_csr_wstream<OP, 64, 512>);
        case CK_WSTREAM_64_1024: PERSIST(k_csr_wstream<OP, 64, 1024>);
        case CK_WSTREAM_32_512:  PERSIST(k_csr_wstream<OP, 32, 512>);
        case CK_WSTREAM_32_1024: PERSIST(k_csr_wstream<OP, 32, 1024>);
        case CK_ROWPAT_0_1: PERSIST(k_csr_rowpat<OP, 0, 1>);
        case CK_ROWPAT_0_2: PERSIST(k_csr_rowpat<OP, 0, 2>);
        case CK_ROWPAT_1_1: PERSIST(k_csr_rowpat<OP, 1, 1>);
        case CK_ROWPAT_1_2: PERSIST(k_csr_rowpat<OP, 1, 2>);
        case CK_ROWPAT_2_1: PERSIST(k_csr_rowpat<OP, 2, 1>);
        case CK_ROWPAT_2_2: PERSIST(k_csr_rowpat<OP, 2, 2>);
        case CK_DICT8_8:  PERSIST(k_csr_dict8<OP, 8>);
        case CK_DICT8_16: PERSIST(k_csr_dict8<OP, 16>);
        case CK_DICT8_24: PERSIST(k_csr_dict8<OP, 24>);
        case CK_ROWPAT4:  PERSIST(k_csr_rowpat4<OP>);
        case CK_ROWPAT5:  return launch_rowpat5<OP>(a);
        case CK_LSTREAM:  PERSIST(k_csr_lstream<OP, 512>);
        case CK_XTILE:    PERSIST(k_csr_xtile<OP>);
        case CK_SELL:     return launch_sell<OP>(M, a);
        case CK_WSTREAM2: PERSIST(k_csr_wstream2<OP>);
        default: break;
    }
#undef PERSIST
    const int W = M.es_W, nc = M.es_nc, lanes = 4 << (p.kernel - CK_ESTREAM_4);
    a.es_wc = M.es_tab; a.es_centry = a.es_wc + W + 1; a.es_crow = a.es_centry + nc + 1; a.es_hw0 = a.es_crow + nc + 1; a.es_np = a.es_hw0 + W;
    a.es_part = M.es_part; a.es_cnt = reinterpret_cast<unsigned*>(M.es_part + 2 * (size_t)W);
    a.es_cbase = M.es_ja16 ? a.es_np + W : nullptr; a.es_ja16 = M.es_ja16;
    static bool attr_set = false;
#define ES_ATTR(LL) (void)hipFuncSetAttribute(reinterpret_cast<const void*>(k_csr_estream<LL, OP>), hipFuncAttributeMaxDynamicSharedMemorySize, ES_LDS_BYTES)
    if (!attr_set) { ES_ATTR(32); ES_ATTR(16); ES_ATTR(8); ES_ATTR(4); attr_set = true; }
#undef ES_ATTR
#define ES_LAUNCH(LL) hipLaunchKernelGGL((k_csr_estream<LL, OP>), dim3(W / 4), dim3(BLOCK), ES_LDS_BYTES, g_ctx.stream, a)
#ifdef FASP_LAB_DEBUG
    if (OP == OP_MXV && g_tune.es_dbg) {
#define ES_DBG(LL, DD) do { (void)hipFuncSetAttribute(reinterpret_cast<const void*>(k_csr_estream<LL, OP_MXV, DD>), hipFuncAttributeMaxDynamicSharedMemorySize, ES_LDS_BYTES); hipLaunchKernelGGL((k_csr_estream<LL, OP_MXV, DD>), dim3(W / 4), dim3(BLOCK), ES_LDS_BYTES, g_ctx.stream, a); } while (0)
        const int dd = g_tune.es_dbg;
        if (lanes == 32) { if (dd == 1) ES_DBG(32, 1); else if (dd == 2) ES_DBG(32, 2); else if (dd == 3) ES_DBG(32, 3); else if (dd == 4) ES_DBG(32, 4); else ES_DBG(32, 7); }
        else if (lanes == 16) { if (dd == 1) ES_DBG(16, 1); else if (dd == 2) ES_DBG(16, 2); else if (dd == 3) ES_DBG(16, 3); else if (dd == 4) ES_DBG(16, 4); else ES_DBG(16, 7); }
        else if (lanes == 8) { if (dd == 1) ES_DBG(8, 1); else if (dd == 2) ES_DBG(8, 2); else if (dd == 3) ES_DBG(8, 3); else if (dd == 4) ES_DBG(8, 4); else ES_DBG(8, 7); }
        else { if (dd == 1) ES_DBG(4, 1); else if (dd == 2) ES_DBG(4, 2); else if (dd == 3) ES_DBG(4, 3); else if (dd == 4) ES_DBG(4, 4); else ES_DBG(4, 7); }
#undef ES_DBG
        return W / 4;
    }
#endif
    static const bool es_log = std::getenv("FASP_HIP_ES_LOG") != nullptr;
    if (es_log) { std::fprintf(stderr, "[es rank %d] op %d rows %d cols %d nnz %d W %d chunks %d lanes %d rel %d x %p y %p b %p\n", comm_rank(), (int)OP, M.row, M.col, M.nnz, W, nc, lanes, M.es_ja16 != nullptr, (const void*)a.x, (void*)a.y, (const void*)a.b); std::fflush(stderr); }
    if (lanes == 32) ES_LAUNCH(32); else if (lanes == 16) ES_LAUNCH(16); else if (lanes == 8) ES_LAUNCH(8); else ES_LAUNCH(4);
#undef ES_LAUNCH
    if (es_log) { const hipError_t e = hipStreamSynchronize(g_ctx.stream); std::fprintf(stderr, "[es rank %d] done: %s\n", comm_rank(), hipGetErrorString(e)); std::fflush(stderr); }
    return W / 4;
}

static void d_mxv(const DevCSR& A, const double* x, double* y)
{
    CsrArgs a{}; a.x = x; a.y = y;
    launch_csr<OP_MXV>(A, a);
}
static void d_resid(const DevCSR& A, const double* x, const double* b, double* y)
{
    CsrArgs a{}; a.x = x; a.y = y; a.b = b;
    launch_csr<OP_RESID>(A, a);
}
static void d_aAxpy(double alpha, const DevCSR& A, const double* x, double* y)
{
    CsrArgs a{}; a.x = x; a.y = y; a.alpha = alpha;
    if (alpha == 1.0) launch_csr<OP_ADD>(A, a);
    else if (alpha == -1.0) launch_csr<OP_SUB>(A, a);
    else launch_csr<OP_AXPY>(A, a);
}

static void d_finalize_to(int G, int nq, unsigned maxmask, double* out, bool dist)
{
    hipLaunchKernelGGL(k_finalize, dim3(1), dim3(BLOCK), 0, g_ctx.stream, g_ctx.d_partials, G, nq,
// ... 50 lines not shown
```

### faspsolver_amd/csrc/hierarchy.hip.h

```cpp

struct DevLevel {
    DevCSR  A, P, R;
    double* diag = nullptr;
    double* l1   = nullptr;
    double *b = nullptr, *xa = nullptr, *xb = nullptr, *w = nullptr;
    double* x  = nullptr;
    double* xo = nullptr;
    bool    x_zero = true;
    bool    presmoothed = false;
    double* halo_pending = nullptr;
    bool    owns_b = true;
    bool    replicated = true;
    int     nloc = 0;
    int     nvec = 0;
    int     row0 = 0;
    int     nglobal = 0;
    std::vector<int> send_off, recv_off;
    int*    d_send_idx = nullptr;
    double* d_sendbuf  = nullptr;
    bool    has_halo() const { return !replicated && nvec > nloc; }
    struct Sched {
        bool built = false, multicolor = false; int* d_order = nullptr; int* d_ptr = nullptr; std::vector<int> ptr;
        int ns = 0, L = 1, LR = 1, pfmax = 1, kt = 0, par = 1, nstrips = 0, nchunk = 0, maxent = 0; bool nolower = false, flow_ok = false, rowlevels = false, independent = false; int nrows = 0, nvirt = 0, nclasses = 0; long long nghost = 0, slot_bytes = 0;
        std::vector<int> cptr;
// ... 213 lines not shown
        (void)launch_csr<OP>(M, a);
        return -1;
    }
    RowWin w;
    w.lo = M.win_lo; w.hi = M.win_hi; w.goff = 0;
    int G = launch_csr<OP>(M, a, w);
    const int hst = halo_exchange(V, v, g_ctx.comm_stream);
    if (hipEventRecord(g_ctx.ev_halo, g_ctx.comm_stream) != hipSuccess ||
        hipStreamWaitEvent(g_ctx.stream, g_ctx.ev_halo, 0) != hipSuccess) {
        comm_mark_failed();
        (void)hipStreamSynchronize(g_ctx.comm_stream);
        local_ok = false;
    }
    w.lo = 0; w.hi = M.win_lo; w.goff = G;
    G += launch_csr<OP>(M, a, w);
    w.lo = M.win_hi; w.hi = M.row; w.goff = G;
    G += launch_csr<OP>(M, a, w);
    return (hst < 0 || !local_ok) ? -1 : G;
}

static bool renumber_param_ok(const AMG_param& p)
{
    return (p.smoother == SMOOTHER_JACOBI || p.smoother == SMOOTHER_L1DIAG) &&
           (p.cycle_type == V_CYCLE || p.cycle_type == W_CYCLE || p.cycle_type == VW_CYCLE || p.cycle_type == WV_CYCLE) &&
           p.coarse_scaling != 1 && p.AMG_type == CLASSIC_AMG;
}
static bool renumber_allowed(const fasp_hip_amg* h)
{
    if (g_oneshot_upload) return false;
    return g_tune.renumber != 0 && comm_size() == 1 && renumber_param_ok(h->param);
}
static int renumber_conflict(const fasp_hip_amg* h, const AMG_param& p)
{
    bool any = false;
    for (const auto& pm : h->perm) any = any || !pm.empty();
    if (!any || renumber_param_ok(p)) return FASP_SUCCESS;
    std::printf("### ERROR: fasp_hip: this hierarchy was uploaded for an order-independent smoother (its mid levels are renumbered); "
                "smoother %d / cycle %d / coarse_scaling %d need the natural order -- set them before the setup, or "
                "fasp_hip_tune(\"renumber\", 0)\n", (int)p.smoother, (int)p.cycle_type, (int)p.coarse_scaling);
    return ERROR_INPUT_PAR;
}
static bool dev_coded(const DevCSR& M) { return M.pat != nullptr || M.code != nullptr; }

static int upload_transfer(fasp_hip_amg* h, int l, const DistLevel* DLp)
{
    const HostLevel& HL = h->H.L[l];
    DevLevel& D = h->L[l];
    const bool rep = !DLp || DLp->replicated;
    const std::vector<int>* pf = (size_t)l < h->perm.size() && !h->perm[(size_t)l].empty() ? &h->perm[(size_t)l] : nullptr;
    const std::vector<int>* pc = (size_t)l + 1 < h->perm.size() && !h->perm[(size_t)l + 1].empty() ? &h->perm[(size_t)l + 1] : nullptr;
    const bool bridged = pc && !pf && dev_coded(D.A);
    if (bridged) {
        if (upload_csr(HL.P, D.P) < 0) return ERROR_ALLOC_MEM;
        if (upload_csr(HL.R, D.R) < 0) return ERROR_ALLOC_MEM;
        DevLevel& C = h->L[(size_t)l + 1];
        if (!C.d_perm) {
            HIPCK(hipMalloc(&C.d_perm, sizeof(int) * pc->size()));
            HIPCK(hipMemcpy(C.d_perm, pc->data(), sizeof(int) * pc->size(), hipMemcpyHostToDevice));
        }
        HIPCK(hipMalloc(&D.R.bscratch, sizeof(double) * pc->size()));
        HIPCK(hipMalloc(&D.P.bscratch, sizeof(double) * pc->size()));
        D.R.bridge = C.d_perm; D.R.bridge_dir = 1;
        D.P.bridge = C.d_perm; D.P.bridge_dir = 2;
    } else if (pf || pc) {
        std::vector<int> invf, invc;
        if (pf) { invf.resize(pf->size()); for (size_t k = 0; k < pf->size(); ++k) invf[(size_t)(*pf)[k]] = (int)k; }
        if (pc) { invc.resize(pc->size()); for (size_t k = 0; k < pc->size(); ++k) invc[(size_t)(*pc)[k]] = (int)k; }
        HostCSR T;
        permute_csr(HL.P, pf ? pf->data() : nullptr, pc ? invc.data() : nullptr, T);
        if (upload_csr(T, D.P) < 0) return ERROR_ALLOC_MEM;
        HIPCK(hipStreamSynchronize(g_ctx.stream));
        permute_csr(HL.R, pc ? pc->data() : nullptr, pf ? invf.data() : nullptr, T);
        if (upload_csr(T, D.R) < 0) return ERROR_ALLOC_MEM;
        HIPCK(hipStreamSynchronize(g_ctx.stream));
    } else {
        if (upload_csr(rep ? HL.P : DLp->P, D.P) < 0) return ERROR_ALLOC_MEM;
        if (upload_csr(rep ? HL.R : DLp->R, D.R) < 0) return ERROR_ALLOC_MEM;
    }
    if (D.A.plane > 0 && D.R.row > 0 && D.R.col > 0) {
        D.P.plane = D.A.plane;
        const long long pr = (long long)D.A.plane * D.R.row;
        if (pr % D.R.col == 0) D.R.plane = (int)(pr / D.R.col);
    }
    if (!rep) {
        D.R.win_lo = DLp->winR[0]; D.R.win_hi = DLp->winR[1];
        D.P.win_lo = DLp->winP[0]; D.P.win_hi = DLp->winP[1];
    }
    return FASP_SUCCESS;
}

static int upload_level(fasp_hip_amg* h, int l, const DistLevel* DLp)
{
    const HostLevel& HL = h->H.L[l];
    DevLevel& D = h->L[l];
    const bool rep = !DLp || DLp->replicated;
    D.replicated = rep;
    D.nloc = rep ? HL.A.row : DLp->nloc; D.row0 = rep ? 0 : DLp->row0; D.nglobal = HL.A.row;
    D.nvec = rep ? HL.A.row : DLp->nloc + (int)DLp->ghosts.size();
    const HostCSR& A = rep ? HL.A : DLp->A;
    static const bool timing = std::getenv("FASP_HIP_SETUP_TIMING") != nullptr;
    double tp = wall_seconds();
    auto lap = [&](const char* what) {
        if (!timing) return;
        const double now = wall_seconds();
        std::printf("    [upload level %d] %-10s %8.3f s\n", l, what, now - tp);
        tp = now;
    };
    const bool renum = renumber_allowed(h);
    if (h->perm.size() < h->L.size()) h->perm.resize(h->L.size());
    HostCSR Aperm;
    const HostCSR* Adev = &A;
    if (!rep && g_tune.local_square) {
        HostCSR view;
        view.row = A.row; view.col = A.col; view.nnz = A.nnz; view.row_aligned = true;
        view.ia.view(const_cast<int*>(A.ia.data()), A.ia.n); view.ja.view(const_cast<int*>(A.ja.data()), A.ja.n); view.val.view(const_cast<double*>(A.val.data()), A.val.n);
        if (upload_csr(view, D.A) < 0) return ERROR_ALLOC_MEM;
    } else {
        bool want = renum && rep && l > 0 && HL.has_coarse && !HL.SWZ && A.row >= 4096 && A.row <= 2000000 && (g_tune.renumber >= 2 || !dev_coded(h->L[(size_t)l - 1].A));
        bool uploaded = false;
        if (want && compress_enabled() && (double)A.nnz <= 48.0 * A.row) {
            if (upload_csr(A, D.A) < 0) return ERROR_ALLOC_MEM;
            if (dev_coded(D.A)) { want = false; uploaded = true; }
            else { HIPCK(hipStreamSynchronize(g_ctx.stream)); D.A.release(); D.A = DevCSR(); }
        }
        if (want) {
            std::vector<int>& pm = h->perm[(size_t)l];
            cluster_order(A, std::max(4096, g_tune.renumber_chunk), pm);
            std::vector<int> inv(pm.size());
            for (size_t k = 0; k < pm.size(); ++k) inv[(size_t)pm[k]] = (int)k;
            permute_csr(A, pm.data(), inv.data(), Aperm);
            Adev = &Aperm;
            lap("renumber");
        }
        if (!uploaded && upload_csr(*Adev, D.A) < 0) return ERROR_ALLOC_MEM;
    }
    lap("A");
    if (renum) {
        if (l > 0 && h->H.L[(size_t)l - 1].has_coarse && !h->L[(size_t)l - 1].P.ia) {
            const int st = upload_transfer(h, l - 1, nullptr);
            if (st < 0) return st;
            lap("P, R of the level above");
        }
    } else if (HL.has_coarse) {
        const int st = upload_transfer(h, l, DLp);
        if (st < 0) return st;
        lap("P, R");
    }
    if (!rep) { D.A.win_lo = DLp->winA[0]; D.A.win_hi = DLp->winA[1]; }
    HIPCK(hipStreamSynchronize(g_ctx.stream));
    lap("sync");
    if (upload_diag(*Adev, D) < 0) return ERROR_ALLOC_MEM;
    lap("diag");
    { const int st = swz_level_upload(h, l); if (st < 0) return st; }
    lap("Schwarz");
    const size_t n = D.nvec;
    if (l > 0) { if (alloc_vec(&D.b, n) < 0) return ERROR_ALLOC_MEM; }
    else D.owns_b = false;
    if (alloc_vec(&D.xa, n) < 0 || alloc_vec(&D.xb, n) < 0 || alloc_vec(&D.w, n) < 0) return ERROR_ALLOC_MEM;
    D.x = D.xa; D.xo = D.xb; D.x_zero = true;
    if (!rep) {
        D.send_off = DLp->send_off; D.recv_off = DLp->recv_off;
        const size_t ns = DLp->send_idx.size();
        HIPCK(hipMalloc(&D.d_send_idx, sizeof(int) * std::max<size_t>(ns, 1)));
        HIPCK(hipMalloc(&D.d_sendbuf, sizeof(double) * std::max<size_t>(ns, 1)));
        if (ns) HIPCK(hipMemcpy(D.d_send_idx, DLp->send_idx.data(), sizeof(int) * ns, hipMemcpyHostToDevice));
    }
// ... 63 lines not shown
```

### faspsolver_amd/csrc/kernels.hip.h

```cpp
#pragma once

#include <hip/hip_runtime.h>

namespace fasp {

constexpr int BLOCK   = 256;
constexpr int MAXGRID = 2048;

enum RowOp : int {
    OP_MXV = 0,
    OP_RESID,
    OP_ADD,
    OP_SUB,
    OP_AXPY,
    OP_JACOBI,
    OP_L1DIAG,
    OP_MXV_DOT
};

struct CsrArgs {
    int           nrow;
    const int*    ia;
    const int*    ja;
    const double* val;
    const double* x;
    double*       y;
    const double* b;
    const double* diag;
    const int*    dpos;
    const double* dotv;
    double*       partials;
    double        alpha;
    double        omega;
    int           ntiles;
    int           tiles_per_xcd;
    int           tpp;
    int           xcd_map;
    int           nt;
    const unsigned char* code;
    const int*    rowbase;
    const int*    doff;
    const double* dval;
    const unsigned short* pat;
    const int*    pstart;
    const int*    plen;
    const int*    poff;
    const double* pval;
    int           npat, npent;
    int           ncol;
    const int*    stop;
    const int*    mark;
    const unsigned short* ja16;
    const int*            jbase;
    int           tile0, row_lo;
    double*       zx;
    const double* zdiag;
    double        zomega;
    const unsigned short* lja16;
    const int*    tptr;
    const int*    tcols;
    const int*    es_wc;
    const int*    es_centry;
    const int*    es_crow;
    const int*    es_hw0;
    const int*    es_np;
    const int*    es_cbase;
    const unsigned short* es_ja16;
    double*       es_part;
    unsigned*     es_cnt;
    const unsigned*      sell_code;
    const int*           sell_sptr;
    const int*           sell_sbase;
    const unsigned char* sell_rlen;
    const double*        sell_tab;
    int                  sell_nv, sell_obits;
};

__device__ __forceinline__ void zx_store(const CsrArgs& a, int r, double s)
{
    if (a.zx) {
        const double di = a.zdiag[r];
        a.zx[r] = (fabs(di) > 1e-20) ? (1 - a.zomega) * 0.0 + a.zomega * s / di : 0.0;
    }
}

__device__ __forceinline__ double l1_or_jacobi_f(const CsrArgs& a, int r, double t, double d, double xi)
{
    if (a.mark) return a.mark[r] == 0 ? xi + a.omega * t / d : xi;
    return (fabs(d) > 1e-20) ? xi + t / d : xi;
}

__device__ __forceinline__ int ld_ja(const CsrArgs& a, int k)
{
    if (a.ja16) return a.nt ? (int)__builtin_nontemporal_load(a.ja16 + k) : (int)a.ja16[k];
    return a.nt ? __builtin_nontemporal_load(a.ja + k) : a.ja[k];
}
__device__ __forceinline__ double ld_val(const CsrArgs& a, int k)
{
    return a.nt ? __builtin_nontemporal_load(a.val + k) : a.val[k];
}
__device__ __forceinline__ int tile_vmax(const CsrArgs& a)
{
    if (a.xcd_map == -2) return 8 * a.tiles_per_xcd * ((a.ntiles + a.tpp - 1) / a.tpp);
    if (a.xcd_map < 0) return 8 * a.tiles_per_xcd;
    if (a.xcd_map <= 0) return a.ntiles;
    const int span = 8 * a.xcd_map;
    return (a.ntiles + span - 1) / span * span;
}
__device__ __forceinline__ int tile_of(const CsrArgs& a, int v)
{
    if (a.xcd_map == -2) {
        const int q = v >> 3, z = q / a.tiles_per_xcd;
        return z * a.tpp + (v & 7) * a.tiles_per_xcd + (q - z * a.tiles_per_xcd);
    }
    if (a.xcd_map < 0) return (v & 7) * a.tiles_per_xcd + (v >> 3);
    if (a.xcd_map <= 0) return v;
    const int G = a.xcd_map;
    const int xcd = v & 7, q = v >> 3;
    int chunk, within;
    if ((G & (G - 1)) == 0) { const int sh = __ffs(G) - 1; chunk = q >> sh; within = q & (G - 1); }
    else { chunk = q / G; within = q - chunk * G; }
    return (chunk * 8 + xcd) * G + within;
}

template <int W>
__device__ __forceinline__ double subwave_sum(double v)
{
#pragma unroll
    for (int off = W / 2; off > 0; off >>= 1) v += __shfl_down(v, off, W);
    return v;
}

__device__ __forceinline__ void wave_lds_sync()
{
    __builtin_amdgcn_fence(__ATOMIC_RELEASE, "workgroup");
    __builtin_amdgcn_wave_barrier();
    __builtin_amdgcn_fence(__ATOMIC_ACQUIRE, "workgroup");
}

__device__ __forceinline__ double block_sum(double v, double* lds )
{
    v = subwave_sum<64>(v);
    const int wave = threadIdx.x >> 6, lane = threadIdx.x & 63;
    __syncthreads();
    if (lane == 0) lds[wave] = v;
    __syncthreads();
    double r = 0.0;
    if (threadIdx.x == 0) r = ((lds[0] + lds[1]) + lds[2]) + lds[3];
    return r;
}
__device__ __forceinline__ double block_max(double v, double* lds)
{
#pragma unroll
    for (int off = 32; off > 0; off >>= 1) v = fmax(v, __shfl_down(v, off, 64));
    const int wave = threadIdx.x >> 6, lane = threadIdx.x & 63;
    __syncthreads();
    if (lane == 0) lds[wave] = v;
    __syncthreads();
    double r = 0.0;
    if (threadIdx.x == 0) r = fmax(fmax(lds[0], lds[1]), fmax(lds[2], lds[3]));
    return r;
}

template <int L, int OP>
__global__ __launch_bounds__(BLOCK) void k_csr_rows(CsrArgs a)
{
    if (a.stop && *a.stop) return;
    constexpr int RPB = BLOCK / L;
    const int sl   = threadIdx.x & (L - 1);
    const int rloc = threadIdx.x / L;
    const int vmax = tile_vmax(a);
    double acc = 0.0;

    for (int v = blockIdx.x; v < vmax; v += gridDim.x) {
        const int t = tile_of(a, v);
        if (t >= a.ntiles) continue;
        const int r = (t + a.tile0) * RPB + rloc;
        if (r < a.nrow) {
            const int kb = a.ia[r], ke = a.ia[r + 1];
            const int jb = a.jbase ? a.jbase[r] : 0;
            double s = 0.0;
            int k = kb + sl;
            for (; k + 3 * L < ke; k += 4 * L) {
                const int    c0 = jb + ld_ja(a, k);
                const int    c1 = jb + ld_ja(a, k + L);
                const int    c2 = jb + ld_ja(a, k + 2 * L);
                const int    c3 = jb + ld_ja(a, k + 3 * L);
                const double v0 = ld_val(a, k);
                const double v1 = ld_val(a, k + L);
                const double v2 = ld_val(a, k + 2 * L);
                const double v3 = ld_val(a, k + 3 * L);
                const double x0 = a.x[c0], x1 = a.x[c1], x2 = a.x[c2], x3 = a.x[c3];
                if (OP == OP_JACOBI) {
// ... 144 lines not shown
                        else if (OP == OP_L1DIAG) acc -= pr;
                        else acc += pr;
                    }
                }
            }
            const double s = acc;
            if (OP == OP_MXV) { a.y[r] = s; zx_store(a, r, s); }
            else if (OP == OP_RESID) a.y[r] = a.b[r] - s;
            else if (OP == OP_ADD) a.y[r] += s;
            else if (OP == OP_SUB) a.y[r] -= s;
            else if (OP == OP_AXPY) a.y[r] += s * a.alpha;
            else if (OP == OP_JACOBI) {
                const double d = a.diag[r], xi = a.x[r];
                a.y[r] = (fabs(d) > 1e-20) ? (1 - a.omega) * xi + a.omega * s / d : xi;
            } else if (OP == OP_L1DIAG) {
                const double d = a.diag[r], xi = a.x[r];
                a.y[r] = l1_or_jacobi_f(a, r, s, d, xi);
            } else if (OP == OP_MXV_DOT) {
                a.y[r] = s;
                dotacc += s * a.dotv[r];
            }
        }
        wave_lds_sync();
        r0A = r0B; nrA = nrB; kbA = kbB; keA = keB; k0A = k0B; k1A = k1B; s0A = s0B; qA0 = qB0; qA1 = qB1;
        r0B = r0C; nrB = nrC; kbB = kbC; keB = keC;
    }
    if (OP == OP_MXV_DOT) {
        const double tot = block_sum(dotacc, red);
        if (threadIdx.x == 0) a.partials[blockIdx.x] = tot;
    }
}

typedef unsigned int u32x2_t __attribute__((ext_vector_type(2)));
__device__ __forceinline__ double buf_load_f64(__amdgpu_buffer_rsrc_t rs, unsigned byte_off)
{
    const u32x2_t v = __builtin_amdgcn_raw_buffer_load_b64(rs, (int)byte_off, 0, 0);
    return __builtin_bit_cast(double, v);
}

template <int OP, int LDS_TAB, int RPL>
__global__ __launch_bounds__(BLOCK) void k_csr_rowpat(CsrArgs a)
{
    if (a.stop && *a.stop) return;
    constexpr int U = 8;
    constexpr int MAXP = LDS_TAB == 2 ? 64 : 512, MAXE = LDS_TAB == 2 ? 512 : 2048;
    __shared__ int    s_start[LDS_TAB ? MAXP : 1];
    __shared__ int    s_len[LDS_TAB ? MAXP : 1];
    __shared__ int    s_off[LDS_TAB ? MAXE : 1];
    __shared__ double s_val[LDS_TAB ? MAXE : 1];
    __shared__ double red[4];
    if (LDS_TAB) {
        for (int i = threadIdx.x; i < a.npat; i += BLOCK) { s_start[i] = a.pstart[i]; s_len[i] = a.plen[i]; }
        for (int i = threadIdx.x; i < a.npent; i += BLOCK) { s_off[i] = a.poff[i]; s_val[i] = a.pval[i]; }
        __syncthreads();
    }
    const int*    pstart = LDS_TAB ? s_start : a.pstart;
    const int*    plen   = LDS_TAB ? s_len : a.plen;
    const int*    poff   = LDS_TAB ? s_off : a.poff;
    const double* pval   = LDS_TAB ? s_val : a.pval;
    const __amdgpu_buffer_rsrc_t xr =
        __builtin_amdgcn_make_buffer_rsrc(const_cast<double*>(a.x), 0, (int)((unsigned)a.ncol * 8u), 0x00020000);
    const int vmax = tile_vmax(a);
    const int G = gridDim.x;
    const int last = a.nrow - 1;
    double dotacc = 0.0;

    auto advance = [&](int& v) -> int {
        for (;;) {
            if (v >= vmax) return -1;
            const int t = tile_of(a, v);
            v += G;
            if (t < a.ntiles) return (t + a.tile0) * (BLOCK * RPL);
        }
    };
    int      v = blockIdx.x;
    int      rA[RPL], cbA[RPL];
    unsigned pidA[RPL];
    int      r0A = advance(v);
#pragma unroll
    for (int q = 0; q < RPL; ++q) {
        rA[q] = max(r0A, 0) + q * BLOCK + (int)threadIdx.x;
        const int rc = min(rA[q], last);
        pidA[q] = a.pat[rc];
        cbA[q] = a.rowbase ? a.rowbase[rc] : rc;
    }
    while (r0A >= 0) {
        const int r0B = advance(v);
        int      rB[RPL], cbB[RPL];
        unsigned pidB[RPL];
#pragma unroll
        for (int q = 0; q < RPL; ++q) {
            rB[q] = max(r0B, 0) + q * BLOCK + (int)threadIdx.x;
            const int rc = min(rB[q], last);
            pidB[q] = a.pat[rc];
            cbB[q] = a.rowbase ? a.rowbase[rc] : rc;
        }
        int    ps[RPL], len[RPL], self[RPL];
        double acc[RPL], dg[RPL], xi[RPL];
#pragma unroll
        for (int q = 0; q < RPL; ++q) {
            const int rc = min(rA[q], last);
            ps[q] = pstart[pidA[q]]; len[q] = plen[pidA[q]];
            self[q] = rc - cbA[q];
            acc[q] = dg[q] = xi[q] = 0.0;
            if (OP == OP_JACOBI || OP == OP_L1DIAG) { acc[q] = a.b[rc]; dg[q] = a.diag[rc]; xi[q] = a.x[rc]; }
        }
        int kmax = len[0];
#pragma unroll
        for (int q = 1; q < RPL; ++q) kmax = max(kmax, len[q]);
        for (int k = 0; k < kmax; k += U) {
            int    off[RPL][U];
            double xv[RPL][U];
#pragma unroll
            for (int q = 0; q < RPL; ++q)
#pragma unroll
                for (int u = 0; u < U; ++u) off[q][u] = (k < len[q]) ? poff[ps[q] + k + u] : 0;
#pragma unroll
            for (int q = 0; q < RPL; ++q)
#pragma unroll
                for (int u = 0; u < U; ++u) xv[q][u] = buf_load_f64(xr, (unsigned)(cbA[q] + off[q][u]) * 8u);
#pragma unroll
            for (int q = 0; q < RPL; ++q)
#pragma unroll
                for (int u = 0; u < U; ++u) {
                    const double pr = ((k < len[q]) ? pval[ps[q] + k + u] : 0.0) * xv[q][u];
                    bool use = k + u < len[q];
                    if (OP == OP_JACOBI) use = use && off[q][u] != self[q];
                    const double nxt = (OP == OP_JACOBI || OP == OP_L1DIAG) ? acc[q] - pr : acc[q] + pr;
                    acc[q] = use ? nxt : acc[q];
                }
        }
#pragma unroll
        for (int q = 0; q < RPL; ++q) {
            if (rA[q] > last) continue;
            const int    r = rA[q];
            const double s = acc[q];
            if (OP == OP_MXV) { a.y[r] = s; zx_store(a, r, s); }
            else if (OP == OP_RESID) a.y[r] = a.b[r] - s;
            else if (OP == OP_ADD) a.y[r] += s;
            else if (OP == OP_SUB) a.y[r] -= s;
            else if (OP == OP_AXPY) a.y[r] += s * a.alpha;
            else if (OP == OP_JACOBI) a.y[r] = (fabs(dg[q]) > 1e-20) ? (1 - a.omega) * xi[q] + a.omega * s / dg[q] : xi[q];
            else if (OP == OP_L1DIAG) a.y[r] = l1_or_jacobi_f(a, r, s, dg[q], xi[q]);
            else if (OP == OP_MXV_DOT) {
                a.y[r] = s;
                dotacc += s * a.dotv[r];
            }
        }
        r0A = r0B;
#pragma unroll
        for (int q = 0; q < RPL; ++q) { rA[q] = rB[q]; pidA[q] = pidB[q]; cbA[q] = cbB[q]; }
    }
    if (OP == OP_MXV_DOT) {
        const double tot = block_sum(dotacc, red);
        if (threadIdx.x == 0) a.partials[blockIdx.x] = tot;
    }
}


template <int OP, int RW, int CAPW>
__global__ __launch_bounds__(BLOCK) void k_csr_wstream(CsrArgs a)
{
    if (a.stop && *a.stop) return;
    __shared__ double prod_all[4 * CAPW];
    const int lane = threadIdx.x & 63, wave = threadIdx.x >> 6;
    double* prod = prod_all + wave * CAPW;

    const int vmax = tile_vmax(a);
    double dotacc = 0.0;

    for (int v = blockIdx.x; v < vmax; v += gridDim.x) {
        const int t = tile_of(a, v);
        if (t >= a.ntiles) continue;
        const int r0 = ((t + a.tile0) * 4 + wave) * RW;
        if (r0 >= a.nrow) continue;
        const int nr = min(RW, a.nrow - r0);
        int kb = 0, ke = 0;
        if (lane < nr) {
// ... 628 lines not shown
```

### faspsolver_amd/csrc/kernels2.hip.h

```cpp
#pragma once

#include "kernels.hip.h"

namespace fasp {

typedef int    i32x4_t __attribute__((ext_vector_type(4)));
typedef double f64x2_t __attribute__((ext_vector_type(2)));
typedef unsigned int u32x4_t __attribute__((ext_vector_type(4)));

__device__ __forceinline__ void wave_order()
{
    __builtin_amdgcn_fence(__ATOMIC_RELEASE, "wavefront");
    __builtin_amdgcn_wave_barrier();
    __builtin_amdgcn_fence(__ATOMIC_ACQUIRE, "wavefront");
}

template <int OP>
__device__ __forceinline__ void row_epilogue(const CsrArgs& a, int r, double s, double& dotacc)
{
    if (OP == OP_MXV) { if (a.nt & 2) __builtin_nontemporal_store(s, a.y + r); else a.y[r] = s; zx_store(a, r, s); }
    else if (OP == OP_RESID) a.y[r] = a.b[r] - s;
    else if (OP == OP_ADD) a.y[r] += s;
    else if (OP == OP_SUB) a.y[r] -= s;
    else if (OP == OP_AXPY) a.y[r] += s * a.alpha;
// ... 600 lines not shown
        else if (OP == OP_RESID) { out.x = bb.x - accA; out.y = bb.y - accB; }
        else if (OP == OP_ADD) { out.x = aux.x + accA; out.y = aux.y + accB; }
        else if (OP == OP_SUB) { out.x = aux.x - accA; out.y = aux.y - accB; }
        else if (OP == OP_AXPY) { out.x = aux.x + accA * a.alpha; out.y = aux.y + accB * a.alpha; }
        else if (OP == OP_JACOBI) {
            if (dg == 0.0) {
                const f64x2_t xi = *reinterpret_cast<const f64x2_t*>(a.x + rs);
                xiA = xi.x; xiB = xi.y;
            }
            out.x = (fabs(dg) > 1e-20) ? (1 - a.omega) * xiA + a.omega * accA / dg : xiA;
            out.y = (fabs(dg) > 1e-20) ? (1 - a.omega) * xiB + a.omega * accB / dg : xiB;
            if (a.partials && mine) { dotacc += out.x * bb.x; dotacc += out.y * bb.y; }
        } else if (OP == OP_L1DIAG) {
            const f64x2_t xi = *reinterpret_cast<const f64x2_t*>(a.x + rs);
            out.x = l1_or_jacobi_f(a, rs, accA, aux.x, xi.x);
            out.y = l1_or_jacobi_f(a, rs + 1, accB, aux.y, xi.y);
        } else {
            out.x = accA; out.y = accB;
            if (mine) { dotacc += accA * aux.x; dotacc += accB * aux.y; }
        }
        if (mine) { pend_out = out; pend_off = (unsigned)ra * 8u; }
        {
            const bool ex = ra <= last && !mine;
            const unsigned long long exm = __ballot(ex);
            if (exm) {
                const int pos = qn + 2 * __popcll(exm & ((1ull << lane) - 1ull));
                if (ex) { myq[pos] = ra; myq[pos + 1] = (ra + 1 <= last) ? ra + 1 : -1; }
                qn += 2 * __popcll(exm);
                while (qn >= 64) drain(64);
            }
        }
        r0A = r0B;
        pp = ppB;
    }
    flush();

    if (qn > 0) drain(qn);
    if (OP == OP_MXV_DOT || (OP == OP_JACOBI && a.partials)) {
        const double tot = block_sum(dotacc, red);
        if (threadIdx.x == 0) a.partials[blockIdx.x] = tot;
    }
}

template <int OP>
__global__ __launch_bounds__(BLOCK) void k_csr_rowpat5(CsrArgs a)
{
    if (a.stop && *a.stop) return;
    static_assert(OP != OP_JACOBI && OP != OP_L1DIAG, "transfer operators are not smoothed");
    __shared__ double red[4];
    __shared__ int xq[4 * RP_QCAP];
    int* const myq = xq + (threadIdx.x >> 6) * RP_QCAP;
    int        qn = 0;
    const int  lane = threadIdx.x & 63;
    const bool stream = (a.nt & 4) != 0;
    const __amdgpu_buffer_rsrc_t xr =
        __builtin_amdgcn_make_buffer_rsrc(const_cast<double*>(a.x), 0, (int)((unsigned)a.ncol * 8u), 0x00020000);
    const __amdgpu_buffer_rsrc_t yr =
        __builtin_amdgcn_make_buffer_rsrc(a.y, 0, (int)((unsigned)(a.nrow & ~1) * 8u), 0x00020000);
    typedef const __attribute__((address_space(4))) int    cint_t;
    typedef const __attribute__((address_space(4))) double cdbl_t;
    cint_t* cpstart = (cint_t*)(a.pstart);
    cint_t* cplen   = (cint_t*)(a.plen);
    cint_t* cpoff   = (cint_t*)(a.poff);
    cdbl_t* cpval   = (cdbl_t*)(a.pval);
    const int vmax = tile_vmax(a);
    const int G = gridDim.x;
    const int last = a.nrow - 1;
    const unsigned* pat2 = reinterpret_cast<const unsigned*>(a.pat);
    const int npair = (a.nrow + 1) >> 1;
    double dotacc = 0.0;

    auto advance = [&](int& v) -> int {
        for (;;) {
            if (v >= vmax) return -1;
            const int t = tile_of(a, v);
            v += G;
            if (t < a.ntiles) return (t + a.tile0) * (2 * BLOCK);
        }
    };
    auto pair_of = [&](int r0) -> int { return min((max(r0, 0) >> 1) + (int)threadIdx.x, npair - 1); };
    auto one_row = [&](int r) {
        const unsigned pid = a.pat[r];
        const int      ps = a.pstart[pid], len = a.plen[pid];
        const unsigned base = (unsigned)a.rowbase[r] * 8u;
        double acc = 0.0;
        for (int k = 0; k < len; k += 8) {
            int    of[8];
            double xk[8];
#pragma unroll
            for (int u = 0; u < 8; ++u) of[u] = a.poff[ps + k + u];
#pragma unroll
            for (int u = 0; u < 8; ++u) xk[u] = buf_load_f64(xr, base + (unsigned)(of[u] * 8));
#pragma unroll
            for (int u = 0; u < 8; ++u) {
                const double pr = a.pval[ps + k + u] * xk[u];
                acc = (k + u < len) ? acc + pr : acc;
            }
        }
        row_epilogue<OP>(a, r, acc, dotacc);
    };
    auto drain = [&](int n) {
        wave_order();
        const int r = lane < n ? myq[qn - n + lane] : -1;
        if (r >= 0) one_row(r);
        qn -= n;
    };
    int      v = blockIdx.x;
    int      r0A = advance(v);
    unsigned pp = stream ? __builtin_nontemporal_load(pat2 + pair_of(r0A)) : pat2[pair_of(r0A)];
    f64x2_t  pend_out = {0.0, 0.0};
    unsigned pend_off = 0xfffffff0u;
    auto flush = [&]() {
        if (stream) __builtin_amdgcn_raw_buffer_store_b128(__builtin_bit_cast(u32x4_t, pend_out), yr, (int)pend_off, 0, 2);
        else __builtin_amdgcn_raw_buffer_store_b128(__builtin_bit_cast(u32x4_t, pend_out), yr, (int)pend_off, 0, 0);
        pend_off = 0xfffffff0u;
    };
    auto sweep_lists = [&](int psA, int lenA, unsigned baseA8, double& accA, int psB, int lenB, unsigned baseB8, double& accB) {
        const int lmax = max(lenA, lenB);
        for (int k = 0; k < lmax; k += 8) {
            const bool doA = k < lenA, doB = k < lenB;
            int    ofA[8], ofB[8];
            double xa[8], xb[8];
#pragma unroll
            for (int u = 0; u < 8; ++u) { ofA[u] = doA ? cpoff[psA + k + u] : 0; ofB[u] = doB ? cpoff[psB + k + u] : 0; }
            const int nA = doA ? min(lenA - k, 8) : 0, nB = doB ? min(lenB - k, 8) : 0;
#pragma unroll
            for (int u = 0; u < 8; ++u) {
                xa[u] = 0.0;
                if (u < nA) xa[u] = buf_load_f64(xr, baseA8 + (unsigned)(ofA[u] * 8));
            }
#pragma unroll
            for (int u = 0; u < 8; ++u) {
                xb[u] = 0.0;
                if (u < nB) xb[u] = buf_load_f64(xr, baseB8 + (unsigned)(ofB[u] * 8));
            }
            if (k == 0) flush();
            auto chunk = [&](int ps, int len, const double (&xv)[8], double& acc) {
                double w[8];
#pragma unroll
                for (int u = 0; u < 8; ++u) w[u] = cpval[ps + k + u];
                auto entry = [&](int u) { acc += w[u] * xv[u]; };
                switch (min(len - k, 8)) {
                    case 8: entry(0); entry(1); entry(2); entry(3); entry(4); entry(5); entry(6); entry(7); break;
                    case 7: entry(0); entry(1); entry(2); entry(3); entry(4); entry(5); entry(6); break;
                    case 6: entry(0); entry(1); entry(2); entry(3); entry(4); entry(5); break;
                    case 5: entry(0); entry(1); entry(2); entry(3); entry(4); break;
                    case 4: entry(0); entry(1); entry(2); entry(3); break;
                    case 3: entry(0); entry(1); entry(2); break;
                    case 2: entry(0); entry(1); break;
                    default: entry(0); break;
                }
            };
            if (doA) chunk(psA, lenA, xa, accA);
            if (doB) chunk(psB, lenB, xb, accB);
        }
        if (lmax == 0) flush();
    };
    while (r0A >= 0) {
        const int      r0B = advance(v);
        const unsigned ppB = stream ? __builtin_nontemporal_load(pat2 + pair_of(r0B)) : pat2[pair_of(r0B)];
        const int  ra = r0A + 2 * (int)threadIdx.x;
        const bool vb = ra + 1 <= last;
        const unsigned pidA = pp & 0xffffu, pidB = pp >> 16;
        const unsigned domA = (unsigned)__builtin_amdgcn_readlane((int)pidA, 32);
        unsigned       domB = (unsigned)__builtin_amdgcn_readlane((int)pidB, 32);
        const bool     domok = domB < (unsigned)a.npat;
        if (!domok) domB = 0;
        const bool     mine = vb && domok && pidA == domA && pidB == domB;
        const int      rs = mine ? ra : 0;
        const int      psA = cpstart[domA], lenA = cplen[domA], psB = cpstart[domB], lenB = cplen[domB];
        const int2 cb = *reinterpret_cast<const int2*>(a.rowbase + rs);
        f64x2_t aux = {0.0, 0.0};
        if (OP == OP_RESID) aux = *reinterpret_cast<const f64x2_t*>(a.b + rs);
        else if (OP == OP_MXV_DOT) aux = *reinterpret_cast<const f64x2_t*>(a.dotv + rs);
        else if (OP == OP_ADD || OP == OP_SUB || OP == OP_AXPY) aux = *reinterpret_cast<const f64x2_t*>(a.y + rs);
        double accA = 0.0, accB = 0.0;
        sweep_lists(psA, lenA, (unsigned)cb.x * 8u, accA, psB, lenB, (unsigned)cb.y * 8u, accB);
        f64x2_t out = {0.0, 0.0};
        if (OP == OP_MXV) { out.x = accA; out.y = accB; if (mine) { zx_store(a, ra, accA); zx_store(a, ra + 1, accB); } }
        else if (OP == OP_RESID) { out.x = aux.x - accA; out.y = aux.y - accB; }
        else if (OP == OP_ADD) { out.x = aux.x + accA; out.y = aux.y + accB; }
        else if (OP == OP_SUB) { out.x = aux.x - accA; out.y = aux.y - accB; }
        else if (OP == OP_AXPY) { out.x = aux.x + accA * a.alpha; out.y = aux.y + accB * a.alpha; }
        else {
            out.x = accA; out.y = accB;
            if (mine) { dotacc += accA * aux.x; dotacc += accB * aux.y; }
        }
        if (mine) { pend_out = out; pend_off = (unsigned)ra * 8u; }
        {
            const bool ex = ra <= last && !mine;
            const unsigned long long exm = __ballot(ex);
            if (exm) {
                const int pos = qn + 2 * __popcll(exm & ((1ull << lane) - 1ull));
                if (ex) { myq[pos] = ra; myq[pos + 1] = (ra + 1 <= last) ? ra + 1 : -1; }
                qn += 2 * __popcll(exm);
                while (qn >= 64) drain(64);
            }
        }
        r0A = r0B;
        pp = ppB;
    }
    flush();

    if (qn > 0) drain(qn);
    if (OP == OP_MXV_DOT) {
        const double tot = block_sum(dotacc, red);
        if (threadIdx.x == 0) a.partials[blockIdx.x] = tot;
    }
}

__global__ __launch_bounds__(BLOCK) void k_copy16(size_t n16, const f64x2_t* __restrict__ src, f64x2_t* __restrict__ dst)
{
    for (size_t i = (size_t)blockIdx.x * BLOCK + threadIdx.x; i < n16; i += (size_t)gridDim.x * BLOCK) dst[i] = src[i];
}
__global__ __launch_bounds__(BLOCK) void k_triad16(size_t n16, double s, const f64x2_t* __restrict__ b,
                                                   const f64x2_t* __restrict__ c, f64x2_t* __restrict__ out)
{
    for (size_t i = (size_t)blockIdx.x * BLOCK + threadIdx.x; i < n16; i += (size_t)gridDim.x * BLOCK) {
        const f64x2_t bv = b[i], cv = c[i];
        f64x2_t o;
        o.x = bv.x + s * cv.x;
        o.y = bv.y + s * cv.y;
        out[i] = o;
    }
}
__global__ __launch_bounds__(BLOCK) void k_read16(size_t n16, const f64x2_t* __restrict__ src, double* __restrict__ out)
{
    double acc = 0.0;
    for (size_t i = (size_t)blockIdx.x * BLOCK + threadIdx.x; i < n16; i += (size_t)gridDim.x * BLOCK) {
        const f64x2_t v = src[i];
        acc += v.x + v.y;
    }
    if (acc == 1.2345e-300) out[0] = acc;
}

}
```

### faspsolver_amd/csrc/solver.hip

```cpp
#include <hip/hip_runtime.h>

#include <fcntl.h>
#include <omp.h>
#include <sys/mman.h>
#include <sys/stat.h>
#include <unistd.h>

#include <algorithm>
#include <cfloat>
#include <cmath>
#include <cstdio>
#include <cstdlib>
#include <cstring>
#include <functional>
#include <condition_variable>
#include <memory>
#include <mutex>
#include <string>
#include <thread>
#include <type_traits>
#include <vector>

#include "fasp_comm.h"
#include "fasp_internal.h"
#include "krylov_ws.h"
#include "kernels.hip.h"
#include "kernels2.hip.h"
#include "kernels3.hip.h"
#include "kernels4.hip.h"
#include "small_solvers.hip.h"
#include "seq_split.hip.h"
#include "seq_chain.hip.h"

namespace fasp_str { struct CsrSwzDev; }

namespace fasp {

#define HIPCK(expr)                                                                        \
    do {                                                                                   \
        hipError_t e_ = (expr);                                                            \
        if (e_ != hipSuccess) {                                                            \
            std::fprintf(stderr, "### ERROR: fasp_hip: %s failed: %s [%s:%d]\n", #expr,    \
                         hipGetErrorString(e_), __FILE__, __LINE__);                       \
            return ERROR_MISC;                                                             \
        }                                                                                  \
    } while (0)

struct Ctx {
    bool        ready  = false;
    int         device = -1;
    hipStream_t stream = nullptr;
    hipStream_t comm_stream = nullptr;
    hipEvent_t  ev_ready = nullptr, ev_halo = nullptr;
    double*     d_partials = nullptr;
    double*     d_partials2 = nullptr;
    double*     h_part     = nullptr;
    double*     d_red      = nullptr;
    double*     h_red      = nullptr;
    int         num_cu     = 256;
};
static Ctx g_ctx;
static int g_requested_device = -1;

constexpr int RED_SLOTS = 16;

static int ctx_init()
{
    if (g_ctx.ready) return FASP_SUCCESS;
    int ndev = 0;
    hipError_t e = hipGetDeviceCount(&ndev);
    if (e != hipSuccess || ndev <= 0) {
        std::fprintf(stderr, "### ERROR: fasp_hip: no HIP device available (%s). This library has "
                             "no CPU fallback.\n", e == hipSuccess ? "device count 0" : hipGetErrorString(e));
        return ERROR_MISC;
    }
    int dev = 0;
    if (g_requested_device >= 0) dev = g_requested_device;
    else if (const char* lr = std::getenv("FASP_HIP_DEVICE")) dev = std::atoi(lr);
    if (dev < 0 || dev >= ndev) {
        const char* wrap = std::getenv("FASP_HIP_ALLOW_DEVICE_WRAP");
        if (wrap && std::atoi(wrap) != 0 && dev >= 0) dev = dev % ndev;
        else {
            std::fprintf(stderr, "### ERROR: fasp_hip: device %d requested, %d visible (one process per GPU; "
                                 "FASP_HIP_ALLOW_DEVICE_WRAP=1 shares devices for the shared-memory validation transport)\n", dev, ndev);
            return ERROR_INPUT_PAR;
        }
    }
    HIPCK(hipSetDevice(dev));
    hipDeviceProp_t prop;
    HIPCK(hipGetDeviceProperties(&prop, dev));
    if (std::strncmp(prop.gcnArchName, "gfx950", 6) != 0)
        std::fprintf(stderr, "### WARNING: fasp_hip: device %d is %s; kernels are built for gfx950\n",
// ... 1967 lines not shown
{
    FASP_ENTRY();
    return hipMemcpyFromSymbol(out, HIP_SYMBOL(fasp::g_flow_times), sizeof(unsigned long long) * (size_t)std::min(n, 8192)) == hipSuccess ? 0 : -1;
}
#endif

static int g_time_cold = 0;
int fasp_hip_tune(const char* key, int value)
{
    FASP_ENTRY();
    if (!key) return ERROR_INPUT_PAR;
    if (!std::strcmp(key, "maxgrid")) g_tune.maxgrid = value;
    else if (!std::strcmp(key, "xcd")) g_tune.xcd = value;
    else if (!std::strcmp(key, "gen2")) g_tune.gen2 = value;
    else if (!std::strcmp(key, "ws2_bpc")) g_tune.ws2_bpc = value;
    else if (!std::strcmp(key, "nt")) g_tune.nt = value;
    else if (!std::strcmp(key, "kind")) g_tune.kind = value;
    else if (!std::strcmp(key, "compress")) g_tune.compress = value;
    else if (!std::strcmp(key, "rpl")) g_tune.rpl = value;
    else if (!std::strcmp(key, "lds_tab")) g_tune.lds_tab = value;
    else if (!std::strcmp(key, "xcd_pat")) g_tune.xcd_pat = value;
    else if (!std::strcmp(key, "spcg_batch")) g_tune.spcg_batch = value;
    else if (!std::strcmp(key, "spcg_fused")) g_tune.spcg_fused = value;
    else if (!std::strcmp(key, "spcg_persist")) { g_tune.spcg_persist = value; if (value) g_persist_disabled = false; }
    else if (!std::strcmp(key, "spcg_test_hang")) g_tune.spcg_test_hang = value;
    else if (!std::strcmp(key, "spcg_grid")) g_tune.spcg_grid = value;
    else if (!std::strcmp(key, "small_lds")) g_tune.small_lds = value;
    else if (!std::strcmp(key, "small_onewave")) g_tune.small_onewave = value;
    else if (!std::strcmp(key, "ja16")) g_tune.ja16 = value;
    else if (!std::strcmp(key, "device_sort")) g_device_sort = value;
    else if (!std::strcmp(key, "halo_overlap")) g_halo_overlap = value;
    else if (!std::strcmp(key, "coarse_mode")) g_coarse_mode = value;
    else if (!std::strcmp(key, "coarse_split_min")) g_coarse_split_min = value;
    else if (!std::strcmp(key, "split_rows")) g_tune.split_rows = value;
    else if (!std::strcmp(key, "gs_multicolor")) g_tune.gs_multicolor = value;
    else if (!std::strcmp(key, "seq_flow")) { g_tune.seq_flow = value; if (value) g_flow_disabled = false; }
    else if (!std::strcmp(key, "ilu_smooth_fused")) g_tune.ilu_smooth_fused = value;
    else if (!std::strcmp(key, "swz_run")) g_tune.swz_run = value;
    else if (!std::strcmp(key, "swz_run_width")) g_tune.swz_run_width = value;
    else if (!std::strcmp(key, "ilu_form")) g_tune.ilu_form = value;
    else if (!std::strcmp(key, "str_ilu_form")) g_tune.str_ilu_form = value;
    else if (!std::strcmp(key, "str_ilu_wgs")) g_tune.str_ilu_wgs = value;
    else if (!std::strcmp(key, "str_sweep_form")) g_tune.str_sweep_form = value;
    else if (!std::strcmp(key, "str_sweep_wgs")) g_tune.str_sweep_wgs = value;
    else if (!std::strcmp(key, "seq_strip_kb")) g_tune.seq_strip_kb = value;
    else if (!std::strcmp(key, "seq_jobs")) g_tune.seq_jobs = value;
    else if (!std::strcmp(key, "local_square")) g_tune.local_square = value;
    else if (!std::strcmp(key, "seq_grid")) g_tune.seq_grid = value;
    else if (!std::strcmp(key, "seq_chain")) g_tune.seq_chain = value;
    else if (!std::strcmp(key, "seq_chain_n1")) g_tune.seq_chain_n1 = value;
    else if (!std::strcmp(key, "seq_chain_grid")) g_tune.seq_chain_grid = value;
    else if (!std::strcmp(key, "seq_test_hang")) g_tune.seq_test_hang = value;
    else if (!std::strcmp(key, "seq_rest_lanes")) g_tune.seq_rest_lanes = value;
    else if (!std::strcmp(key, "seq_chain_ref")) g_tune.seq_chain_ref = value;
    else if (!std::strcmp(key, "seq_spine")) g_tune.seq_spine = value;
    else if (!std::strcmp(key, "seq_partition")) g_seq_partition = value;
    else if (!std::strcmp(key, "fuse_zr")) g_tune.fuse_zr = value;
    else if (!std::strcmp(key, "fuse_presmooth")) g_tune.fuse_presmooth = value;
    else if (!std::strcmp(key, "seq_lanes")) g_tune.seq_lanes = value;
    else if (!std::strcmp(key, "lazy_coarse")) g_tune.lazy_coarse = value;
    else if (!std::strcmp(key, "xtile")) g_tune.xtile = value;
    else if (!std::strcmp(key, "rp5_max")) g_tune.rp5_max = value;
    else if (!std::strcmp(key, "rp_bpc")) g_tune.rp_bpc = value;
    else if (!std::strcmp(key, "rp_stream")) g_tune.rp_stream = value;
    else if (!std::strcmp(key, "renumber")) g_tune.renumber = value;
    else if (!std::strcmp(key, "renumber_chunk")) g_tune.renumber_chunk = value;
    else if (!std::strcmp(key, "time_cold")) g_time_cold = value;
    else if (!std::strcmp(key, "estream")) g_tune.estream = value;
    else if (!std::strcmp(key, "sell")) g_tune.sell = value;
    else if (!std::strcmp(key, "es_dbg")) g_tune.es_dbg = value;
    else if (!std::strcmp(key, "pcg_dev_beta")) g_tune.pcg_dev_beta = value;
    else if (!std::strcmp(key, "seq_chain_touch")) g_tune.seq_chain_touch = value;
    else if (!std::strcmp(key, "seq_chain_touch_t1")) g_tune.seq_chain_touch_t1 = value;
    else if (!std::strcmp(key, "seq_zero_skip")) g_tune.seq_zero_skip = value;
    else if (!std::strcmp(key, "pcg_fold")) g_tune.pcg_fold = value;
    else if (!std::strcmp(key, "spcg_spec")) g_tune.spcg_spec = value;
    else if (!std::strcmp(key, "ev_every")) g_tune.ev_every = value;
    else if (!std::strcmp(key, "rp_xcd")) g_tune.rp_xcd = value;
    else if (!std::strcmp(key, "rp_strip")) g_tune.rp_strip = value;
    else if (!std::strcmp(key, "host_parallel_min")) g_parallel_min_nnz = value;
    else if (!std::strcmp(key, "rap_form")) g_rap_form = value;
    else if (!std::strcmp(key, "rap_arena_kb")) g_rap_arena_kb = value;
    else if (!std::strcmp(key, "device_rap")) g_device_rap = value;
    else if (!std::strcmp(key, "lanes")) g_tune.lanes = value;
    else if (!std::strcmp(key, "wrows")) g_tune.wrows = value;
    else if (!std::strcmp(key, "wcap")) g_tune.wcap = value;
    else return ERROR_INPUT_PAR;
    return FASP_SUCCESS;
}

int fasp_hip_sell_selftest(const dCSRmat* A, int cap_percent, int* info, double* bytes, int* ia_out, int* ja_out, double* val_out, const double* x, double* y)
{
    if (!A || !info || A->row < 0 || A->nnz < 0) return ERROR_INPUT_PAR;
    HostCSR M;
    M.row = A->row; M.col = A->col; M.nnz = A->nnz;
    M.ia.view(A->IA, (size_t)A->row + 1); M.ja.view(A->JA, (size_t)std::max(A->nnz, 1)); M.val.view(A->val, (size_t)std::max(A->nnz, 1));
    SellHost S;
    int why = 0;
    const bool ok = build_sell(M, S, cap_percent > 0 ? cap_percent : SELL_CAP_PERCENT, &why);
    info[0] = ok ? 1 : 0; info[1] = why; info[2] = S.nv; info[3] = S.vbits; info[4] = S.obits; info[5] = S.nslice;
    info[6] = ok ? (int)std::min<long long>(S.slots / 64, 0x7fffffff) : 0; info[7] = SELL_MAXV;
    if (bytes) *bytes = ok ? S.bytes(M.row) : 0.0;
    if (!ok) return FASP_SUCCESS;
    if (ia_out && ja_out && val_out) sell_decode_host(S, M.row, ia_out, ja_out, val_out);
    if (x && y) sell_mxv_host(S, M.row, x, y);
    return FASP_SUCCESS;
}

int fasp_hip_csr_plan(const int* traits, int op, int windowed, int want_partials, int* plan, double* bytes)
{
    FASP_ENTRY();
    if (!traits || !plan || op < OP_MXV || op > OP_MXV_DOT) return ERROR_INPUT_PAR;
    static double dummy[1];
    const int* t = traits;
    auto flag = [&](int i) -> void* { return t[i] ? dummy : nullptr; };
    DevCSR M;
    M.row = t[0]; M.col = t[1]; M.nnz = t[2]; M.kind = t[3]; M.lanes = t[4]; M.wrows = t[5]; M.wcap = t[6]; M.nxrows = t[7]; M.plane = t[8];
    M.npat = t[9]; M.npent = t[10]; M.sell_nv = t[11]; M.sell_nslice = t[12]; M.sell_slots = t[13]; M.ntcols = t[14]; M.es_W = t[15]; M.es_nc = t[16];
    M.code = (unsigned char*)flag(17); M.pat = (unsigned short*)flag(18); M.rowbase = (int*)flag(19); M.dpos = (int*)flag(20); M.dup_diag = t[21] != 0;
    M.ja16 = (unsigned short*)flag(22); M.jbase = (int*)flag(23); M.lja16 = (unsigned short*)flag(24); M.sell_code = (unsigned*)flag(25);
    M.es_tab = (int*)flag(26); M.es_ja16 = (unsigned short*)flag(27);
    const CsrPlan p = plan_csr(M, op, windowed || g_tune.split_rows > 0, want_partials != 0);
    const int out[11] = {(int)p.kernel, p.family, p.tile_rows, p.bpc, p.xcd_map, p.tpp, p.nt, p.ja16, p.jbase, p.fused_zr, kernel_family(M, nullptr)};
    std::copy(out, out + 11, plan);
    if (bytes) *bytes = p.bytes;
    return FASP_SUCCESS;
}

int fasp_hip_estream_selftest(const int* ia, int nrow, int nnz, int per_wave, int wmax, int* info)
{
    if (!ia || nrow < 1 || nnz < 1 || per_wave < 8 || wmax < 32) return ERROR_INPUT_PAR;
    return estream_selftest_host(ia, nrow, nnz, per_wave, wmax, info);
}

int fasp_hip_measure_ceilings(double* out, size_t bytes, int reps)
{
    FASP_ENTRY();
    if (!out || bytes < (1u << 20) || reps <= 0) return ERROR_INPUT_PAR;
    if (ctx_init() != FASP_SUCCESS) return ERROR_MISC;
    f64x2_t *p = nullptr, *q = nullptr, *r = nullptr;
    HIPCK(hipMalloc(&p, bytes)); HIPCK(hipMalloc(&q, bytes)); HIPCK(hipMalloc(&r, bytes));
    HIPCK(hipMemsetAsync(p, 0, bytes, g_ctx.stream)); HIPCK(hipMemsetAsync(q, 0, bytes, g_ctx.stream));
    HIPCK(hipMemsetAsync(r, 0, bytes, g_ctx.stream));
    const size_t n16 = bytes / 16;
    hipEvent_t e0, e1;
    HIPCK(hipEventCreate(&e0)); HIPCK(hipEventCreate(&e1));
    const int grid = 4 * g_ctx.num_cu;
    for (int which = 0; which < 3; ++which) {
        auto run = [&]() {
            if (which == 0) hipLaunchKernelGGL(k_read16, dim3(grid), dim3(BLOCK), 0, g_ctx.stream, n16, p, (double*)q);
            else if (which == 1) hipLaunchKernelGGL(k_copy16, dim3(grid), dim3(BLOCK), 0, g_ctx.stream, n16, p, q);
            else hipLaunchKernelGGL(k_triad16, dim3(grid), dim3(BLOCK), 0, g_ctx.stream, n16, 0.5, p, q, r);
        };
        run(); run();
        HIPCK(hipEventRecord(e0, g_ctx.stream));
        for (int i = 0; i < reps; ++i) run();
        HIPCK(hipEventRecord(e1, g_ctx.stream));
        HIPCK(hipEventSynchronize(e1));
        float ms = 0.f;
        HIPCK(hipEventElapsedTime(&ms, e0, e1));
        out[which] = (double)(which + 1) * (double)bytes * reps / ((double)ms * 1e-3) / 1e9;
    }
    (void)hipEventDestroy(e0); (void)hipEventDestroy(e1);
    (void)hipFree(p); (void)hipFree(q); (void)hipFree(r);
    return FASP_SUCCESS;
}

double fasp_hip_time_kernel(fasp_hip_amg* h, int kind, int level, int reps)
{
    FASP_ENTRY();
    if (!h || level < 0 || level >= (int)h->L.size() || reps <= 0) return -1.0;
    DevLevel& D = h->L[level];
    const int n = D.A.row;
    hipEvent_t e0, e1;
    if (hipEventCreate(&e0) != hipSuccess || hipEventCreate(&e1) != hipSuccess) return -1.0;
    double* x = D.xa; double* y = D.xb; double* w = D.w;
    auto run = [&]() {
        switch (kind) {
            case 0: d_mxv(D.A, x, y); break;
            case 1: d_aAxpy(-1.0, D.A, x, y); break;
            case 2: { CsrArgs a{}; a.x = x; a.y = y; a.b = w; a.diag = D.diag; a.omega = 0.6667; launch_csr<OP_JACOBI>(D.A, a); } break;
            case 3: hipLaunchKernelGGL(k_dot, dim3(vec_grid(n)), dim3(BLOCK), 0, g_ctx.stream, n, x, y, g_ctx.d_partials); break;
            case 4: d_axpy(n, 0.5, x, y); break;
            case 5: { CsrArgs a{}; a.x = x; a.y = y; a.dotv = x; a.partials = g_ctx.d_partials; launch_csr<OP_MXV_DOT>(D.A, a); } break;
            case 6: if (D.R.ia) d_mxv(D.R, w, h->L[level + 1].xa); break;
            case 7: if (D.P.ia) d_aAxpy(1.0, D.P, h->L[level + 1].xa, y); break;
            case 8:
                if (D.A.val) hipLaunchKernelGGL(k_read16, dim3(2048), dim3(BLOCK), 0, g_ctx.stream, (size_t)D.A.nnz / 2, (const f64x2_t*)D.A.val, y);
                break;
            case 10: case 11: case 12: case 13: (void)seq_sweep(h, level, kind - 10, 1, 1.0); break;
            default: break;
        }
    };
    (void)hipMemsetAsync(x, 0, sizeof(double) * n, g_ctx.stream);
    (void)hipMemsetAsync(y, 0, sizeof(double) * n, g_ctx.stream);
    (void)hipMemsetAsync(w, 0, sizeof(double) * n, g_ctx.stream);
    double* const keep_b = D.b; double* const keep_x = D.x;
    if (kind >= 10) { D.b = w; D.x = x; }
    if (g_time_cold) {
        double* big = nullptr;
        const size_t bigb = (size_t)512 << 20;
        if (hipMalloc(&big, bigb + 4096) != hipSuccess) return -1.0;
        (void)hipMemsetAsync(big, 0, bigb, g_ctx.stream);
        double tot = 0.0;
        for (int i = 0; i < reps + 1; ++i) {
            if (g_time_cold >= 2) (void)hipMemsetAsync(big, 0, bigb, g_ctx.stream);
            else hipLaunchKernelGGL(k_read16, dim3(1024), dim3(BLOCK), 0, g_ctx.stream, bigb / 16, (const f64x2_t*)big, big + bigb / 8);
            (void)hipEventRecord(e0, g_ctx.stream);
// ... 173 lines not shown
```

### include/fasp_hip_dev.h

```cpp
#ifndef FASP_HIP_DEV_H
#define FASP_HIP_DEV_H
#include "fasp_hip.h"
#ifdef __cplusplus
extern "C" {
#endif

double fasp_hip_time_kernel(fasp_hip_amg* h, int kind, int level, int reps);
double fasp_hip_time_matrix(const dCSRmat* A, int op, int reps, int* kind_out);
double fasp_hip_seq_schedule_selftest(const dCSRmat* A, const int* seq, int ns, int strip_kb, int lanes, int spine, int* info);
int fasp_hip_cluster_order(const dCSRmat* A, int chunk, int* order);
int fasp_hip_permute_csr(const dCSRmat* A, const int* rperm, const int* cinv, int* ia, int* ja, double* val);
double fasp_hip_seq_chain_selftest(const dCSRmat* A, const int* seq, int ns, int n1_blocks, int form, double w, int* info, double* out_u);
int fasp_hip_measure_ceilings(double* out, size_t bytes, int reps);

int    fasp_hip_ilu_resident_count(void);
double fasp_hip_ilu_time(ILU_data* iludata, int which, int reps, double* info);
int    fasp_hip_bsr_amg_get_ilu(const fasp_hip_amg_bsr* h, int level, ILU_data* view);
int    fasp_hip_bsr_amg_ilu_info(const fasp_hip_amg_bsr* h, int level, double info[6]);
double fasp_hip_bsr_amg_ilu_smooth_time(fasp_hip_amg_bsr* h, int level, int reps);

int    fasp_hip_dcsr_rap(const dCSRmat* R, const dCSRmat* A, const dCSRmat* P, dCSRmat* RAP);
int    fasp_hip_rap_info(int info[4]);
long   fasp_hip_rap_device_count(void);
double fasp_hip_rap_time(const dCSRmat* R, const dCSRmat* A, const dCSRmat* P, int where, int reps);

int fasp_hip_tune(const char* key, int value);
int fasp_hip_coarse_kernel_info(const fasp_hip_amg* h, int* info);
int fasp_hip_bsr_coarse_kernel_info(const fasp_hip_amg_bsr* h, int* info);

int fasp_hip_comm_stats(double* out8, int reset);
int fasp_hip_comm_timing(int on);

int fasp_hip_dist_plan(fasp_hip_amg* h, int rank, int nranks, int min_rows);
int fasp_hip_dist_level_info(const fasp_hip_amg* h, int level, int* info);
int fasp_hip_dist_get_matrix(const fasp_hip_amg* h, int level, int which, dCSRmat* view);
int fasp_hip_dist_get_list(const fasp_hip_amg* h, int level, int which, ivector* view);
int  fasp_hip_estream_selftest(const int* ia, int nrow, int nnz, int per_wave, int wmax, int* info);
int  fasp_hip_csr_plan(const int* traits, int op, int windowed, int want_partials, int* plan, double* bytes);
int  fasp_hip_sell_selftest(const dCSRmat* A, int cap_percent, int* info, double* bytes, int* ia_out, int* ja_out, double* val_out, const double* x, double* y);
int  fasp_hip_level_op(fasp_hip_amg* h, int level, int which, int op, const double* x, const double* b, double* y, double* y2, double scalar, double* red);
int  fasp_hip_matrix_op(const dCSRmat* A, int op, const double* x, const double* b, double* y, double* y2, double scalar, double* red, int* kind_out);
int  fasp_hip_matrix_traits(const dCSRmat* A, int* traits);
int  fasp_hip_bsr_sweep(const dBSRmat* A, const double* b, double* u, const double* diaginv, int descend, int sor, double w, int* nlevels);
int  fasp_hip_csr_sweep(const dCSRmat* A, const int* seq, int ns, int form, double w, int zero_start, const double* b, double* u, int* info);
int  fasp_hip_str_form(const dSTRmat* A);
double fasp_hip_time_str_mxv(const dSTRmat* A, int reps);
int    fasp_hip_str_ilu_form(const dSTRmat* LU, int lfil);
int    fasp_hip_str_ilu_apply(const dSTRmat* LU, int lfil, const double* r, double* z);
double fasp_hip_time_str_ilu(const dSTRmat* LU, int lfil, int reps);
int    fasp_hip_str_sweep(const dSTRmat* A, int kind, int order, const int* mark, double weight, const double* diaginv, const double* b,
                          double* u, int nsweeps, int* info);
int    fasp_hip_str_sweep_form(const dSTRmat* A, int order, const int* mark);
int    fasp_hip_str_sweep_levels(const dSTRmat* A, int order, const int* mark, int* visit, int* level, int cap);
double fasp_hip_time_str_sweep(const dSTRmat* A, int kind, int order, const int* mark, double weight, int reps);
int  fasp_hip_str_swz(const dSTRmat* A, const int* neigh, int nneigh, const int* order, const double* b, double* u, int nsweeps, int* info);
int  fasp_hip_str_swz_levels(const dSTRmat* A, const int* neigh, int nneigh, const int* order, int* visit, int* level, int cap);
int  fasp_hip_time_str_swz(const dSTRmat* A, const int* neigh, int nneigh, const int* order, int reps, double* ms_factor, double* ms_sweep, int* info);
int  fasp_hip_csr_swz_levels(const SWZ_data* swz, int backward, int* level, int cap);
int  fasp_hip_csr_swz(SWZ_data* swz, int dir, const double* b, double* x, int nsweeps, int* info, double* fac, int* piv);
int  fasp_hip_csr_swz_resident_count(void);
int  fasp_hip_time_csr_swz(SWZ_data* swz, int reps, double* ms, double* bytes, int* info);
int    fasp_hip_csr_swz_runs(const SWZ_data* swz, int backward, int width, int* run_first, int cap);
int    fasp_hip_amg_get_swz(const fasp_hip_amg* h, int level, SWZ_data* view);
int    fasp_hip_amg_swz_levels(const fasp_hip_amg* h, int level, int* swz_levels);
int    fasp_hip_amg_swz_info(const fasp_hip_amg* h, int level, int* info);
double fasp_hip_amg_swz_sweep_time(fasp_hip_amg* h, int level, int dir, int reps);
int  fasp_hip_comm_selftest(void);

#ifdef __cplusplus
}
#endif
#endif
```

Measured before the change: 480.8 million.

## Add column-plane-aware tile scheduling table for R/P transfers and optional 16-bit rowbase

Builds a per-matrix tile table for the restriction and prolongation operators that groups row tiles by the column-plane strip they read and interleaves them across the 8 XCD slots. The SpMV kernels then fetch tiles through that table (xcd_map -3) so each XCD keeps touching a nearby slice of the input vector, aiming to improve L2 locality. The table is enabled by default. Separately, rowbase offsets can be compressed into a 16-bit delta plus a 64-row group base to cut index bytes, but that path is off by default. Costs are extra host setup, an indirect tile lookup in the kernel, and padding entries in the table.

```diff
diff --git a/faspsolver_amd/__init__.py b/faspsolver_amd/__init__.py
--- a/faspsolver_amd/__init__.py
+++ b/faspsolver_amd/__init__.py
@@ -39,7 +39,7 @@
     "fasp_hip_dist_get_list",
     "fasp_blas_dcsr_vmv", "fasp_blas_dcsr_mxv_agg", "fasp_blas_dcsr_aAxpy_agg", "fasp_blas_darray_ax",
     "fasp_blas_darray_axpyz", "fasp_blas_darray_norm1", "fasp_darray_cp", "fasp_darray_set", "fasp_dvec_isnan",
-    "fasp_hip_time_matrix", "fasp_hip_bsr_dist_info", "fasp_hip_seq_schedule_selftest", "fasp_hip_seq_chain_selftest", "fasp_hip_cluster_order", "fasp_hip_permute_csr", "fasp_hip_comm_init_ipc", "fasp_hip_comm_stats", "fasp_hip_comm_timing", "fasp_hip_estream_selftest", "fasp_hip_sell_selftest", "fasp_hip_csr_plan", "fasp_hip_level_op", "fasp_hip_matrix_op", "fasp_hip_matrix_traits",
+    "fasp_hip_time_matrix", "fasp_hip_bsr_dist_info", "fasp_hip_seq_schedule_selftest", "fasp_hip_seq_chain_selftest", "fasp_hip_cluster_order", "fasp_hip_permute_csr", "fasp_hip_comm_init_ipc", "fasp_hip_comm_stats", "fasp_hip_comm_timing", "fasp_hip_estream_selftest", "fasp_hip_sell_selftest", "fasp_hip_csr_plan", "fasp_hip_tile_table", "fasp_hip_amg_tile_info", "fasp_hip_rowbase16_selftest", "fasp_hip_level_op", "fasp_hip_matrix_op", "fasp_hip_matrix_traits",
     "fasp_param_ilu_init", "fasp_ilu_data_create", "fasp_ilu_data_free", "fasp_mem_iludata_check", "fasp_ilu_dcsr_setup",
     "fasp_precond_ilu", "fasp_precond_ilu_forward", "fasp_precond_ilu_backward", "fasp_solver_dcsr_krylov_ilu",
     "fasp_solver_dcsr_krylov_ilu_M", "fasp_smoother_dcsr_ilu", "fasp_fwrapper_dcsr_krylov_ilu_",
@@ -165,6 +165,9 @@
     L.fasp_fwrapper_dcsr_krylov_amg_.restype = None
     L.fasp_hip_coding_selftest.argtypes = [P(T.dCSRmat), P(C.c_int)]
     L.fasp_hip_amg_kernel_info.argtypes = [C.c_void_p, C.c_int, C.c_int, P(C.c_int), P(C.c_double)]
+    L.fasp_hip_amg_tile_info.argtypes = [C.c_void_p, C.c_int, C.c_int, P(C.c_int)]
+    L.fasp_hip_rowbase16_selftest.argtypes = [P(C.c_int), C.c_int, P(C.c_int)]
+    L.fasp_hip_tile_table.argtypes = [P(T.dCSRmat), C.c_int, C.c_int, C.c_int, P(C.c_int), C.c_int, P(C.c_int)]
     L.fasp_hip_coarse_kernel_info.argtypes = [C.c_void_p, P(C.c_int)]
     L.fasp_hip_bsr_coarse_kernel_info.argtypes = [C.c_void_p, P(C.c_int)]
     L.fasp_solver_amg.argtypes = [P(T.dCSRmat), P(T.dvector), P(T.dvector), P(T.AMG_param)]
@@ -595,6 +598,12 @@
             raise IndexError((level, which))
         return k.value, b.value
 
+    def tile_info(self, level, which=0):
+        info = (C.c_int * 8)()
+        if lib().fasp_hip_amg_tile_info(self.h, level, which, info) < 0:
+            raise IndexError((level, which))
+        return dict(zip(("xcd_map", "tile_len", "tile_tab_rows", "colplane", "why", "tile_rows", "rb16", "rb16_coded"), list(info)))
+
     def coarse_kernel_info(self):
         info = (C.c_int * 8)()
         if lib().fasp_hip_coarse_kernel_info(self.h, info) < 0:
diff --git a/faspsolver_amd/csrc/device_csr.hip.h b/faspsolver_amd/csrc/device_csr.hip.h
--- a/faspsolver_amd/csrc/device_csr.hip.h
+++ b/faspsolver_amd/csrc/device_csr.hip.h
@@ -43,8 +43,17 @@
     double*        sell_tab = nullptr;
     int            sell_nv = 0, sell_obits = 0, sell_nslice = 0;
     long long      sell_slots = 0;
+    unsigned short* rb16 = nullptr;
+    int*    rbgrp = nullptr;
+    int*    tile_tab = nullptr;
+    int     tile_len = 0, tile_tab_rows = 0, tile_colplane = 0, tile_why = 1;
     void    release()
     {
+        if (rb16) (void)hipFree(rb16);
+        if (rbgrp) (void)hipFree(rbgrp);
+        rb16 = nullptr; rbgrp = nullptr;
+        if (tile_tab) (void)hipFree(tile_tab);
+        tile_tab = nullptr; tile_len = tile_tab_rows = tile_colplane = 0; tile_why = 1;
         if (sell_code) (void)hipFree(sell_code);
         if (sell_meta) (void)hipFree(sell_meta);
         if (sell_rlen) (void)hipFree(sell_rlen);
@@ -338,6 +347,52 @@
     return best;
 }
 
+static bool encode_rowbase16(const int* rb, int n, std::vector<int>& grp, std::vector<unsigned short>& d16)
+{
+    const int ng = (n + 63) / 64;
+    grp.assign((size_t)std::max(ng, 0), 0); d16.assign((size_t)std::max(n, 0), 0);
+    bool fits = true;
+#pragma omp parallel for schedule(static) reduction(&& : fits)
+    for (int g = 0; g < ng; ++g) {
+        const int r0 = g * 64, r1 = std::min(n, r0 + 64);
+        int lo = rb[r0];
+        for (int r = r0; r < r1; ++r) lo = std::min(lo, rb[r]);
+        grp[(size_t)g] = lo;
+        for (int r = r0; r < r1; ++r) {
+            const long long d = (long long)rb[r] - lo;
+            if (d > 65535) fits = false;
+            d16[(size_t)r] = (unsigned short)d;
+        }
+    }
+    return fits;
+}
+
+static bool build_tile_table(const int* ia, const int* ja, int nrow, int tile_rows, int colplane, bool any_size, std::vector<int>& tab)
+{
+    tab.clear();
+    if (nrow < 1 || tile_rows < 1 || colplane < 1) return false;
+    const int ntiles = (nrow + tile_rows - 1) / tile_rows, strip = std::max(1, colplane / 8);
+    std::vector<int> cmin((size_t)ntiles);
+#pragma omp parallel for schedule(static)
+    for (int t = 0; t < ntiles; ++t) {
+        const int r0 = t * tile_rows, r1 = (int)std::min<long long>((long long)r0 + tile_rows, nrow);
+        int c = INT_MAX;
+        for (int k = ia[r0]; k < ia[r1]; ++k) c = std::min(c, ja[k]);
+        cmin[(size_t)t] = c == INT_MAX ? 0 : std::max(c, 0);
+    }
+    std::vector<int> list[8];
+    for (int t = 0; t < ntiles; ++t) list[std::min(7, cmin[(size_t)t] % colplane / strip)].push_back(t);
+    size_t longest = 0;
+    for (auto& l : list) {
+        std::stable_sort(l.begin(), l.end(), [&](int x, int y) { return cmin[(size_t)x] < cmin[(size_t)y]; });
+        longest = std::max(longest, l.size());
+    }
+    tab.assign(8 * longest, -1);
+    for (int s = 0; s < 8; ++s)
+        for (size_t k = 0; k < list[s].size(); ++k) tab[8 * k + (size_t)s] = list[s][k];
+    return any_size || (double)tab.size() <= 1.125 * ntiles + 8.0;
+}
+
 static bool rows_span_16bit(const int* ia, const int* ja, int row)
 {
     int bad = 0;
@@ -861,6 +916,7 @@
     return FASP_SUCCESS;
 }
 
+static bool rowbase16_enabled();
 static int upload_csr(const HostCSR& H, DevCSR& D)
 {
     D.row = H.row; D.col = H.col; D.nnz = H.nnz;
@@ -895,6 +951,13 @@
             if (prb.n) {
                 HIPCK(hipMalloc(&D.rowbase, sizeof(int) * ((size_t)H.row + 2)));
                 HIPCK(hipMemcpy(D.rowbase, prb.data(), sizeof(int) * (size_t)H.row, hipMemcpyHostToDevice));
+                std::vector<int> grp; std::vector<unsigned short> d16;
+                if (rowbase16_enabled() && encode_rowbase16(prb.data(), H.row, grp, d16)) {
+                    HIPCK(hipMalloc(&D.rb16, sizeof(unsigned short) * ((size_t)H.row + 2)));
+                    HIPCK(hipMalloc(&D.rbgrp, sizeof(int) * (grp.size() + 1)));
+                    HIPCK(hipMemcpy(D.rb16, d16.data(), sizeof(unsigned short) * (size_t)H.row, hipMemcpyHostToDevice));
+                    HIPCK(hipMemcpy(D.rbgrp, grp.data(), sizeof(int) * grp.size(), hipMemcpyHostToDevice));
+                }
                 const int nr = H.row, npair = (nr + 1) / 2;
                 long long nx = 0;
 #pragma omp parallel for schedule(static) reduction(+ : nx)
@@ -1005,8 +1068,9 @@
     return build_estream(H.ia.data(), H.row, H.nnz, D);
 }
 
-struct Tuning { int swz_run = -1, swz_run_width = 16, ilu_smooth_fused = 1, gen2 = 2, ws2_bpc = 3, maxgrid = -1, xcd = 16, nt = 1, kind = -1, lanes = -1, wrows = -1, wcap = -1, compress = 1, rpl = -1, lds_tab = 1, xcd_pat = 64, spcg_batch = 16, small_lds = 1, ja16 = 1, spcg_fused = 1, spcg_grid = 0, spcg_persist = 1, split_rows = 0, gs_multicolor = 0, seq_flow = 1, seq_strip_kb = 0, seq_jobs = 1, seq_spine = 1, seq_grid = 0, seq_chain = 1, seq_chain_n1 = 0, seq_chain_grid = 0, seq_chain_ref = 0, seq_test_hang = 0, seq_rest_lanes = 0, local_square = 1, fuse_zr = 1, fuse_presmooth = 1, seq_lanes = 0, xtile = 1, rp5_max = 45, rp_bpc = 5, rp_xcd = -1, rp_strip = 2, spcg_test_hang = 0, small_onewave = 4, lazy_coarse = 1, rp_stream = -1, renumber = 1, renumber_chunk = 262144, pcg_dev_beta = 1, spcg_spec = 1, ev_every = 4, pcg_fold = 1, seq_chain_touch = 8, seq_chain_touch_t1 = 1, seq_zero_skip = 1, estream = 1, es_dbg = 0, ilu_form = -1, str_ilu_form = -1, str_ilu_wgs = 0, str_sweep_form = -1, str_sweep_wgs = 0, sell = 1; };
+struct Tuning { int swz_run = -1, swz_run_width = 16, ilu_smooth_fused = 1, gen2 = 2, ws2_bpc = 3, maxgrid = -1, xcd = 16, nt = 1, kind = -1, lanes = -1, wrows = -1, wcap = -1, compress = 1, rpl = -1, lds_tab = 1, xcd_pat = 64, spcg_batch = 16, small_lds = 1, ja16 = 1, spcg_fused = 1, spcg_grid = 0, spcg_persist = 1, split_rows = 0, gs_multicolor = 0, seq_flow = 1, seq_strip_kb = 0, seq_jobs = 1, seq_spine = 1, seq_grid = 0, seq_chain = 1, seq_chain_n1 = 0, seq_chain_grid = 0, seq_chain_ref = 0, seq_test_hang = 0, seq_rest_lanes = 0, local_square = 1, fuse_zr = 1, fuse_presmooth = 1, seq_lanes = 0, xtile = 1, rp5_max = 45, rp_bpc = 5, rp_xcd = -1, rp_strip = 2, spcg_test_hang = 0, small_onewave = 4, lazy_coarse = 1, rp_stream = -1, renumber = 1, renumber_chunk = 262144, pcg_dev_beta = 1, spcg_spec = 1, ev_every = 4, pcg_fold = 1, seq_chain_touch = 8, seq_chain_touch_t1 = 1, seq_zero_skip = 1, estream = 1, es_dbg = 0, ilu_form = -1, str_ilu_form = -1, str_ilu_wgs = 0, str_sweep_form = -1, str_sweep_wgs = 0, sell = 1, tile_tab = 1, rowbase16 = 0; };
 static Tuning g_tune;
+static bool rowbase16_enabled() { return g_tune.rowbase16 != 0; }
 
 template <class K>
 static int resident_blocks_per_cu(K kernel)
@@ -1051,6 +1115,7 @@
     int    tpp;
     int    nt;
     bool   ja16, jbase;
+    bool   rb16;
     bool   fused_zr;
     double bytes;
 };
@@ -1078,7 +1143,9 @@
         if (!g_tune.rp_strip || M.plane < 8 * rpb || M.plane % (8 * rpb) != 0 || ntiles() < 4 * (M.plane / rpb)) return;
         p.xcd_map = -2; p.tpp = M.plane / rpb;
     };
-    const double avg = M.row > 0 ? (double)M.nnz / M.row : 1.0, ptr_bytes = 4.0 * (M.row + 1.0), base_bytes = M.rowbase ? 4.0 * M.row : 0.0;
+    const bool rb16 = M.rb16 && g_tune.rowbase16 && kind == 5;
+    const double avg = M.row > 0 ? (double)M.nnz / M.row : 1.0, ptr_bytes = 4.0 * (M.row + 1.0),
+                 base_bytes = !M.rowbase ? 0.0 : rb16 ? 2.0 * M.row + 4.0 * ((M.row + 63) / 64) : 4.0 * M.row;
     const bool pair = kind == 5 && M.nxrows >= 0 && g_tune.rpl <= 0;
     p.bytes = kind == 5 ? 2.0 * M.row + base_bytes + 12.0 * M.npent : kind == 4 ? 1.0 * M.nnz + ptr_bytes + base_bytes : 12.0 * M.nnz + ptr_bytes;
     if (pair && g_tune.gen2 && !M.rowbase) {
@@ -1126,6 +1193,12 @@
         else
             p.kernel = lanes == 2 ? CK_ROWS_2 : lanes == 4 ? CK_ROWS_4 : lanes == 8 ? CK_ROWS_8 : lanes == 16 ? CK_ROWS_16 : lanes == 32 ? CK_ROWS_32 : CK_ROWS_64;
     }
+    p.rb16 = rb16 && M.rowbase && (p.family == 5 || p.family == 9);
+    const bool es_kernel = p.kernel >= CK_ESTREAM_4 && p.kernel <= CK_ESTREAM_32;
+    if (M.tile_tab && g_tune.tile_tab > 0 && !windowed && rows == M.row && p.tile_rows == M.tile_tab_rows && !es_kernel && op != OP_MXV_DOT &&
+        !(jac && want_partials) && (p.xcd_map != -2 || p.kernel == CK_ROWPAT5 || g_tune.tile_tab >= 2)) {
+        p.xcd_map = -3; p.tpp = 0;
+    }
     return p;
 }
 static int kernel_family(const DevCSR& M, double* matrix_bytes)
@@ -1133,6 +1206,24 @@
     const CsrPlan p = plan_csr(M, OP_MXV, false, false);
     if (matrix_bytes) *matrix_bytes = p.bytes;
     return p.family;
+}
+
+static int upload_tile_table(const HostCSR& H, DevCSR& D, int op, int colplane)
+{
+    if (D.tile_tab) { (void)hipFree(D.tile_tab); D.tile_tab = nullptr; }
+    D.tile_len = D.tile_tab_rows = D.tile_colplane = 0; D.tile_why = 1;
+    if (g_tune.tile_tab <= 0 || H.row < 1 || H.nnz < 1) return FASP_SUCCESS;
+    const bool any = g_tune.tile_tab >= 2;
+    if (colplane <= 0 && any) colplane = H.col;
+    if (colplane <= 0) { D.tile_why = 2; return FASP_SUCCESS; }
+    const int rpb = plan_csr(D, op, false, false).tile_rows;
+    std::vector<int> tab;
+    D.tile_colplane = colplane;
+    if (!build_tile_table(H.ia.data(), H.ja.data(), H.row, rpb, colplane, any, tab)) { D.tile_why = 3; return FASP_SUCCESS; }
+    HIPCK(hipMalloc(&D.tile_tab, sizeof(int) * std::max<size_t>(tab.size(), 8)));
+    HIPCK(hipMemcpy(D.tile_tab, tab.data(), sizeof(int) * tab.size(), hipMemcpyHostToDevice));
+    D.tile_len = (int)tab.size(); D.tile_tab_rows = rpb; D.tile_why = 0;
+    return FASP_SUCCESS;
 }
 
 template <int OP>
@@ -1235,11 +1326,13 @@
     a.ntiles = (w_hi - w_lo + rpb - 1) / rpb; a.tiles_per_xcd = (a.ntiles + 7) / 8;
     a.xcd_map = p.xcd_map; a.nt = p.nt;
     if (p.tpp) { a.tpp = p.tpp; a.tiles_per_xcd = p.tpp / 8; }
+    if (p.xcd_map == -3) { a.tile_tab = M.tile_tab; a.tile_len = M.tile_len; }
     a.ia = M.ia; a.ja = M.ja; a.val = M.val; a.dpos = M.dpos;
     a.ja16 = p.ja16 ? M.ja16 : nullptr; a.jbase = p.jbase ? M.jbase : nullptr;
     if (p.family == 5 || p.family == 6 || p.family == 9) {
         a.pat = M.pat; a.pstart = M.pstart; a.plen = M.plen; a.poff = M.poff; a.pval = M.pval; a.rowbase = M.rowbase;
         a.npat = M.npat; a.npent = M.npent; a.ncol = M.col;
+        if (p.rb16) { a.rb16 = M.rb16; a.rbgrp = M.rbgrp; }
     }
     if (p.family == 4) { a.code = M.code; a.rowbase = M.rowbase; a.doff = M.doff; a.dval = M.dval; }
     if (p.kernel == CK_XTILE) { a.lja16 = M.lja16; a.tptr = M.tptr; a.tcols = M.tcols; }
diff --git a/faspsolver_amd/csrc/hierarchy.hip.h b/faspsolver_amd/csrc/hierarchy.hip.h
--- a/faspsolver_amd/csrc/hierarchy.hip.h
+++ b/faspsolver_amd/csrc/hierarchy.hip.h
@@ -319,6 +319,11 @@
         const long long pr = (long long)D.A.plane * D.R.row;
         if (pr % D.R.col == 0) D.R.plane = (int)(pr / D.R.col);
     }
+    if (rep && (bridged || !(pf || pc))) {
+        const int cplane = D.R.plane > 0 ? D.R.plane : (size_t)l + 1 < h->L.size() ? h->L[(size_t)l + 1].A.plane : 0;
+        if (upload_tile_table(HL.R, D.R, OP_MXV, D.A.plane) < 0) return ERROR_ALLOC_MEM;
+        if (upload_tile_table(HL.P, D.P, OP_ADD, cplane) < 0) return ERROR_ALLOC_MEM;
+    }
     if (!rep) {
         D.R.win_lo = DLp->winR[0]; D.R.win_hi = DLp->winR[1];
         D.P.win_lo = DLp->winP[0]; D.P.win_hi = DLp->winP[1];
diff --git a/faspsolver_amd/csrc/kernels.hip.h b/faspsolver_amd/csrc/kernels.hip.h
--- a/faspsolver_amd/csrc/kernels.hip.h
+++ b/faspsolver_amd/csrc/kernels.hip.h
@@ -36,9 +36,13 @@
     int           tiles_per_xcd;
     int           tpp;
     int           xcd_map;
+    const int*    tile_tab;
+    int           tile_len;
     int           nt;
     const unsigned char* code;
     const int*    rowbase;
+    const unsigned short* rb16;
+    const int*    rbgrp;
     const int*    doff;
     const double* dval;
     const unsigned short* pat;
@@ -90,6 +94,10 @@
     return (fabs(d) > 1e-20) ? xi + t / d : xi;
 }
 
+__device__ __forceinline__ int ld_rowbase(const CsrArgs& a, int r)
+{
+    return a.rb16 ? a.rbgrp[r >> 6] + (int)a.rb16[r] : a.rowbase[r];
+}
 __device__ __forceinline__ int ld_ja(const CsrArgs& a, int k)
 {
     if (a.ja16) return a.nt ? (int)__builtin_nontemporal_load(a.ja16 + k) : (int)a.ja16[k];
@@ -99,8 +107,10 @@
 {
     return a.nt ? __builtin_nontemporal_load(a.val + k) : a.val[k];
 }
+typedef const __attribute__((address_space(4))) int* tile_int_cp;
 __device__ __forceinline__ int tile_vmax(const CsrArgs& a)
 {
+    if (a.xcd_map == -3) return a.tile_len;
     if (a.xcd_map == -2) return 8 * a.tiles_per_xcd * ((a.ntiles + a.tpp - 1) / a.tpp);
     if (a.xcd_map < 0) return 8 * a.tiles_per_xcd;
     if (a.xcd_map <= 0) return a.ntiles;
@@ -109,6 +119,10 @@
 }
 __device__ __forceinline__ int tile_of(const CsrArgs& a, int v)
 {
+    if (a.xcd_map == -3) {
+        const int t = ((tile_int_cp)(unsigned long long)a.tile_tab)[v];
+        return t < 0 ? a.ntiles : t;
+    }
     if (a.xcd_map == -2) {
         const int q = v >> 3, z = q / a.tiles_per_xcd;
         return z * a.tpp + (v & 7) * a.tiles_per_xcd + (q - z * a.tiles_per_xcd);
@@ -419,7 +433,7 @@
         rA[q] = max(r0A, 0) + q * BLOCK + (int)threadIdx.x;
         const int rc = min(rA[q], last);
         pidA[q] = a.pat[rc];
-        cbA[q] = a.rowbase ? a.rowbase[rc] : rc;
+        cbA[q] = a.rowbase ? ld_rowbase(a, rc) : rc;
     }
     while (r0A >= 0) {
         const int r0B = advance(v);
@@ -430,7 +444,7 @@
             rB[q] = max(r0B, 0) + q * BLOCK + (int)threadIdx.x;
             const int rc = min(rB[q], last);
             pidB[q] = a.pat[rc];
-            cbB[q] = a.rowbase ? a.rowbase[rc] : rc;
+            cbB[q] = a.rowbase ? ld_rowbase(a, rc) : rc;
         }
         int    ps[RPL], len[RPL], self[RPL];
         double acc[RPL], dg[RPL], xi[RPL];
diff --git a/faspsolver_amd/csrc/kernels2.hip.h b/faspsolver_amd/csrc/kernels2.hip.h
--- a/faspsolver_amd/csrc/kernels2.hip.h
+++ b/faspsolver_amd/csrc/kernels2.hip.h
@@ -706,7 +706,7 @@
     auto one_row = [&](int r) {
         const unsigned pid = a.pat[r];
         const int      ps = a.pstart[pid], len = a.plen[pid];
-        const unsigned base = (unsigned)a.rowbase[r] * 8u;
+        const unsigned base = (unsigned)ld_rowbase(a, r) * 8u;
         double acc = 0.0;
         for (int k = 0; k < len; k += 8) {
             int    of[8];
@@ -793,7 +793,12 @@
         const bool     mine = vb && domok && pidA == domA && pidB == domB;
         const int      rs = mine ? ra : 0;
         const int      psA = cpstart[domA], lenA = cplen[domA], psB = cpstart[domB], lenB = cplen[domB];
-        const int2 cb = *reinterpret_cast<const int2*>(a.rowbase + rs);
+        int2 cb;
+        if (a.rb16) {
+            const unsigned d2 = *reinterpret_cast<const unsigned*>(a.rb16 + rs);
+            const int      g = a.rbgrp[rs >> 6];
+            cb.x = g + (int)(d2 & 0xffffu); cb.y = g + (int)(d2 >> 16);
+        } else cb = *reinterpret_cast<const int2*>(a.rowbase + rs);
         f64x2_t aux = {0.0, 0.0};
         if (OP == OP_RESID) aux = *reinterpret_cast<const f64x2_t*>(a.b + rs);
         else if (OP == OP_MXV_DOT) aux = *reinterpret_cast<const f64x2_t*>(a.dotv + rs);
diff --git a/faspsolver_amd/csrc/solver.hip b/faspsolver_amd/csrc/solver.hip
--- a/faspsolver_amd/csrc/solver.hip
+++ b/faspsolver_amd/csrc/solver.hip
@@ -8,6 +8,7 @@
 
 #include <algorithm>
 #include <cfloat>
+#include <climits>
 #include <cmath>
 #include <cstdio>
 #include <cstdlib>
@@ -2141,6 +2142,8 @@
     else if (!std::strcmp(key, "rap_form")) g_rap_form = value;
     else if (!std::strcmp(key, "rap_arena_kb")) g_rap_arena_kb = value;
     else if (!std::strcmp(key, "device_rap")) g_device_rap = value;
+    else if (!std::strcmp(key, "tile_tab")) g_tune.tile_tab = value;
+    else if (!std::strcmp(key, "rowbase16")) g_tune.rowbase16 = value;
     else if (!std::strcmp(key, "lanes")) g_tune.lanes = value;
     else if (!std::strcmp(key, "wrows")) g_tune.wrows = value;
     else if (!std::strcmp(key, "wcap")) g_tune.wcap = value;
@@ -2183,6 +2186,37 @@
     const int out[11] = {(int)p.kernel, p.family, p.tile_rows, p.bpc, p.xcd_map, p.tpp, p.nt, p.ja16, p.jbase, p.fused_zr, kernel_family(M, nullptr)};
     std::copy(out, out + 11, plan);
     if (bytes) *bytes = p.bytes;
+    return FASP_SUCCESS;
+}
+
+int fasp_hip_tile_table(const dCSRmat* A, int tile_rows, int colplane, int any_size, int* tab, int cap, int* info)
+{
+    if (!A || !info || A->row < 1 || tile_rows < 1 || colplane < 1 || !A->IA || (A->nnz > 0 && !A->JA)) return ERROR_INPUT_PAR;
+    std::vector<int> t;
+    const bool ok = build_tile_table(A->IA, A->JA, A->row, tile_rows, colplane, any_size != 0, t);
+    info[0] = ok ? 1 : 0; info[1] = (int)t.size(); info[2] = (A->row + tile_rows - 1) / tile_rows;
+    if (tab) std::copy(t.begin(), t.begin() + (long)std::min<size_t>(t.size(), (size_t)std::max(cap, 0)), tab);
+    return FASP_SUCCESS;
+}
+int fasp_hip_rowbase16_selftest(const int* rb, int n, int* decoded)
+{
+    if (!rb || n < 1) return ERROR_INPUT_PAR;
+    std::vector<int> grp; std::vector<unsigned short> d16;
+    if (!encode_rowbase16(rb, n, grp, d16)) return 0;
+    if (decoded)
+        for (int r = 0; r < n; ++r) decoded[r] = grp[(size_t)(r >> 6)] + (int)d16[(size_t)r];
+    return 1;
+}
+int fasp_hip_amg_tile_info(const fasp_hip_amg* h, int level, int which, int* info)
+{
+    FASP_ENTRY();
+    if (!h || !info || level < 0 || level >= (int)h->L.size() || which < 0 || which > 2) return ERROR_INPUT_PAR;
+    const DevLevel& D = h->L[level];
+    const DevCSR& M = which == 0 ? D.A : which == 1 ? D.P : D.R;
+    if (!M.ia) return ERROR_INPUT_PAR;
+    const CsrPlan p = plan_csr(M, which == 1 ? OP_ADD : OP_MXV, g_tune.split_rows > 0, false);
+    info[0] = p.xcd_map; info[1] = M.tile_len; info[2] = M.tile_tab_rows; info[3] = M.tile_colplane; info[4] = M.tile_why; info[5] = p.tile_rows;
+    info[6] = p.rb16 ? 1 : 0; info[7] = M.rb16 ? 1 : (M.rowbase && M.pat) ? 0 : -1;
     return FASP_SUCCESS;
 }
 
diff --git a/include/fasp_hip_dev.h b/include/fasp_hip_dev.h
--- a/include/fasp_hip_dev.h
+++ b/include/fasp_hip_dev.h
@@ -37,6 +37,9 @@
 int fasp_hip_dist_get_list(const fasp_hip_amg* h, int level, int which, ivector* view);
 int  fasp_hip_estream_selftest(const int* ia, int nrow, int nnz, int per_wave, int wmax, int* info);
 int  fasp_hip_csr_plan(const int* traits, int op, int windowed, int want_partials, int* plan, double* bytes);
+int  fasp_hip_tile_table(const dCSRmat* A, int tile_rows, int colplane, int any_size, int* tab, int cap, int* info);
+int  fasp_hip_rowbase16_selftest(const int* rb, int n, int* decoded);
+int  fasp_hip_amg_tile_info(const fasp_hip_amg* h, int level, int which, int* info);
 int  fasp_hip_sell_selftest(const dCSRmat* A, int cap_percent, int* info, double* bytes, int* ia_out, int* ja_out, double* val_out, const double* x, double* y);
 int  fasp_hip_level_op(fasp_hip_amg* h, int level, int which, int op, const double* x, const double* b, double* y, double* y2, double scalar, double* red);
 int  fasp_hip_matrix_op(const dCSRmat* A, int op, const double* x, const double* b, double* y, double* y2, double scalar, double* red, int* kind_out);
```

New measurement: 480.9 million (median of 2 runs). Within noise of the previous version (+0.0%).
